# zzbuzzard/PATHS

Measured on AMD Instinct MI355X. Metric: slides_per_sec_5level_K2048_D1024, higher is better.
Workload: dtype f32 (products as 2 fp16 planes per operand = 22 bits, 3 fp16 MFMAs per block, fp32 accumulate); 1 GPU; 5-level PATHS recursion (forward, eval): K=2048 patches/level (level-0 grid 32x64, top_k 512, 10% background), D=1024 features, trans_dim 128 x 4 heads x 2 layers, LSTM ctx 256; 8 HBM-resident slides per GPU; slides_per_gpu=8, global_batch=8, levels=5, resident_batches_rotated=3, parallelism=slide-sharded x1 (no data-path collective)

## Files before the change

### paths_amd/csrc/gemm_epi.h

```cpp
#pragma once
#include "common.h"

namespace paths_epi {



struct TileView {
  char* base; int64_t ldb; uint32_t lane_off;
  __device__ TileView(const float* p, int64_t ld, int lane)
      : base(reinterpret_cast<char*>(const_cast<float*>(p))), ldb(ld * 4), lane_off((uint32_t)((4 * (lane >> 5)) * ld + (lane & 31)) * 4u) {}
  __device__ float* at(int trow, int tcol, int r) const {
    char* tile = base + (int64_t)trow * ldb + (int64_t)tcol * 4;
    const uint32_t off = lane_off + (uint32_t)((r & 3) + 8 * (r >> 2)) * (uint32_t)ldb;
    return reinterpret_cast<float*>(tile + off);
  }
  __device__ char* tile(int trow, int tcol) const { return base + (int64_t)trow * ldb + (int64_t)tcol * 4; }
  __device__ float* elem(char* tile_origin, int r) const {
    return reinterpret_cast<float*>(tile_origin + (lane_off + (uint32_t)((r & 3) + 8 * (r >> 2)) * (uint32_t)ldb));
  }
  __device__ float* at_clamped(int trow, int tcol, int r, int lane, int M) const {
    const int row = min(trow + c32_row(r, lane), M - 1);
    return reinterpret_cast<float*>(base + (int64_t)row * ldb + (int64_t)(tcol + (lane & 31)) * 4);
  }
};
template <bool FULL>
__device__ __forceinline__ float* tile_elem(const TileView& v, int trow, int tcol, int r, int lane, int M) {
  if constexpr (FULL) return v.at(trow, tcol, r);
  else return v.at_clamped(trow, tcol, r, lane, M);
}
template <bool FULL>
__device__ __forceinline__ float* tile_elem_o(const TileView& v, char* origin, int trow, int tcol, int r, int lane, int M) {
  if constexpr (FULL) return v.elem(origin, r);
  else return v.at_clamped(trow, tcol, r, lane, M);
}
template <bool FULL>
__device__ __forceinline__ bool tile_row_ok(int trow, int r, int lane, int M) {
  if constexpr (FULL) return true;
  else return trow + c32_row(r, lane) < M;
}

struct EpiLstmC {
  const float* bias;
  const float* c0; int64_t ldc0;
  float* c1; int64_t ldc1;
  float* frm; int64_t ldfrm;
  const float* hp; int64_t ldhp; const int* hp_row;
  float acc_scale = 1.0f;
  template <int WTM, int WTN>
  __device__ __forceinline__ void init(f32x16 (&acc)[WTM][WTN], int row0, int col0, int lane, int M) const {
    const int jj = lane & 31;
    const float seed = 1.0f / acc_scale;
    if (hp == nullptr) {
#pragma unroll
      for (int i = 0; i < WTM; ++i)
#pragma unroll
        for (int r = 0; r < 16; ++r) { acc[i][0][r] = 0.f; acc[i][1][r] = 0.f; acc[i][2][r] = 0.f; }
      return;
    }
    int pr[WTM][16];
#pragma unroll
    for (int i = 0; i < WTM; ++i)
#pragma unroll
      for (int r = 0; r < 16; ++r) pr[i][r] = hp_row[min(row0 + 32 * i + c32_row(r, lane), M - 1)];
    float t[2][3][16];
    auto issue = [&](auto ic) __attribute__((always_inline)) {
      constexpr int i = decltype(ic)::value;
#pragma unroll
      for (int r = 0; r < 16; ++r) {
        const float* ph = hp + (int64_t)max(pr[i][r], 0) * ldhp + col0 + jj;
        t[i & 1][0][r] = ph[0]; t[i & 1][1][r] = ph[32]; t[i & 1][2][r] = ph[64];
      }
    };
    issue(std::integral_constant<int, 0>{});
    static_for<0, WTM>([&](auto ic) __attribute__((always_inline)) {
      constexpr int i = decltype(ic)::value;
      __builtin_amdgcn_sched_barrier(0);
      if constexpr (i + 1 < WTM) issue(std::integral_constant<int, i + 1>{});
      __builtin_amdgcn_sched_barrier(0);
#pragma unroll
      for (int r = 0; r < 16; ++r) {
        const bool has = pr[i][r] >= 0;
        acc[i][0][r] = has ? t[i & 1][0][r] * seed : 0.f; acc[i][1][r] = has ? t[i & 1][1][r] * seed : 0.f; acc[i][2][r] = has ? t[i & 1][2][r] * seed : 0.f;
      }
    });
    __builtin_amdgcn_sched_barrier(0);
  }
  template <bool FULL, bool WITH_FRM, int WTM, int WTN>
  __device__ __forceinline__ void run_impl(f32x16 (&acc)[WTM][WTN], int row0, int col0, int lane, int M) const {
    const int jj = lane & 31;
    const int tcol = (col0 / 96) * 32;
    const float bf = bias[col0 + jj], br = bias[col0 + 32 + jj], bm = bias[col0 + 64 + jj];
    const TileView c0v(c0, ldc0, lane), c1v(c1, ldc1, lane), fv(frm, ldfrm, lane);
    static_for<0, WTM>([&](auto ic) __attribute__((always_inline)) {
      constexpr int i = decltype(ic)::value;
      const int trow = row0 + 32 * i;
      char* o0 = c0v.tile(trow, tcol); char* o1 = c1v.tile(trow, tcol); char* of = fv.tile(trow, col0);
      float cp[16];
#pragma unroll
      for (int r = 0; r < 16; ++r) cp[r] = c0 ? *tile_elem_o<FULL>(c0v, o0, trow, tcol, r, lane, M) : 0.f;
#pragma unroll
      for (int r = 0; r < 16; ++r) {
        const float f = sigmoid_acc(fmaf(acc[i][0][r], acc_scale, bf));
        const float rg = sigmoid_acc(fmaf(acc[i][1][r], acc_scale, br));
        const float mp = tanh_acc(fmaf(acc[i][2][r], acc_scale, bm));
        const float v = cp[r] * f + rg * mp;
        if (tile_row_ok<FULL>(trow, r, lane, M)) {
          *tile_elem_o<FULL>(c1v, o1, trow, tcol, r, lane, M) = v;
          if constexpr (WITH_FRM) {
            float* fr = tile_elem_o<FULL>(fv, of, trow, col0, r, lane, M);
            fr[0] = f; fr[32] = rg; fr[64] = mp;
          }
        }
      }
      __builtin_amdgcn_sched_barrier(0);
    });
  }
  template <int WTM, int WTN, int WGM, int WGN>
  __device__ __forceinline__ void run(f32x16 (&acc)[WTM][WTN], int row0, int col0, int lane, int, int, int M, float*) const {
    static_assert(WTN == 3, "LSTM c epilogue wants f|r|m tiles");
    const bool full = row0 + 32 * WTM <= M;
    if (frm == nullptr) {
      if (full) run_impl<true, false>(acc, row0, col0, lane, M);
      else run_impl<false, false>(acc, row0, col0, lane, M);
    } else {
      if (full) run_impl<true, true>(acc, row0, col0, lane, M);
      else run_impl<false, true>(acc, row0, col0, lane, M);
    }
  }
};

template <bool RAW>
struct EpiLstmO_ {
  const float* bias; float* o; int64_t ldo; int N;
  const float* hp; int64_t ldhp; const int* hp_row; int hp_col0;
  float acc_scale = 1.0f;
  template <int WTM, int WTN>
  __device__ __forceinline__ void init(f32x16 (&acc)[WTM][WTN], int row0, int col0, int lane, int M) const {
    const float seed = 1.0f / acc_scale;
    if (hp == nullptr) {
#pragma unroll
      for (int i = 0; i < WTM; ++i)
#pragma unroll
        for (int j = 0; j < WTN; ++j)
#pragma unroll
          for (int r = 0; r < 16; ++r) acc[i][j][r] = 0.f;
      return;
    }
    int pr[WTM][16];
#pragma unroll
    for (int i = 0; i < WTM; ++i)
#pragma unroll
      for (int r = 0; r < 16; ++r) pr[i][r] = hp_row[min(row0 + 32 * i + c32_row(r, lane), M - 1)];
    float t[2][WTN][16];
    auto issue = [&](auto ic) __attribute__((always_inline)) {
      constexpr int i = decltype(ic)::value;
#pragma unroll
      for (int r = 0; r < 16; ++r) {
        const float* ph = hp + (int64_t)max(pr[i][r], 0) * ldhp + hp_col0 + (lane & 31);
#pragma unroll
        for (int j = 0; j < WTN; ++j) t[i & 1][j][r] = ph[min(col0 + 32 * j, N - 32)];
      }
    };
    issue(std::integral_constant<int, 0>{});
    static_for<0, WTM>([&](auto ic) __attribute__((always_inline)) {
      constexpr int i = decltype(ic)::value;
      __builtin_amdgcn_sched_barrier(0);
      if constexpr (i + 1 < WTM) issue(std::integral_constant<int, i + 1>{});
      __builtin_amdgcn_sched_barrier(0);
#pragma unroll
      for (int r = 0; r < 16; ++r)
#pragma unroll
        for (int j = 0; j < WTN; ++j) acc[i][j][r] = pr[i][r] >= 0 ? t[i & 1][j][r] * seed : 0.f;
    });
    __builtin_amdgcn_sched_barrier(0);
  }
  template <bool FULL, int WTM, int WTN>
  __device__ __forceinline__ void run_impl(f32x16 (&acc)[WTM][WTN], int row0, int col0, int lane, int M) const {
    const TileView ov(o, ldo, lane);
    static_for<0, WTM * WTN>([&](auto tc) __attribute__((always_inline)) {
      constexpr int t = decltype(tc)::value, i = t % WTM, j = t / WTM;
      const int trow = row0 + 32 * i, tcol = col0 + 32 * j;
      if (tcol < N) {
        const float b = bias[tcol + (lane & 31)];
        char* origin = ov.tile(trow, tcol);
#pragma unroll
        for (int r = 0; r < 16; ++r) {
          const float v = sigmoid_acc(fmaf(acc[i][j][r], acc_scale, b));
          if (tile_row_ok<FULL>(trow, r, lane, M)) *tile_elem_o<FULL>(ov, origin, trow, tcol, r, lane, M) = v;
        }
      }
    });
  }
  template <int WTM, int WTN, int WGM, int WGN>
  __device__ __forceinline__ void run(f32x16 (&acc)[WTM][WTN], int row0, int col0, int lane, int, int, int M, float*) const {
    if constexpr (RAW) {
      const int ntn = N >> 5;
#pragma unroll
      for (int j = 0; j < WTN; ++j) {
        const int tcol = col0 + 32 * j;
        if (tcol < N) {
          const float b = bias[tcol + (lane & 31)];
#pragma unroll
          for (int i = 0; i < WTM; ++i) {
            f32x4* t = reinterpret_cast<f32x4*>(o + ((int64_t)((row0 >> 5) + i) * ntn + (tcol >> 5)) * 1024) + lane;
#pragma unroll
            for (int q = 0; q < 4; ++q)
              t[64 * q] = f32x4{fmaf(acc[i][j][4 * q], acc_scale, b), fmaf(acc[i][j][4 * q + 1], acc_scale, b),
                                fmaf(acc[i][j][4 * q + 2], acc_scale, b), fmaf(acc[i][j][4 * q + 3], acc_scale, b)};
          }
        }
      }
    } else {
      if (row0 + 32 * WTM <= M) run_impl<true>(acc, row0, col0, lane, M);
      else run_impl<false>(acc, row0, col0, lane, M);
    }
  }
};
typedef EpiLstmO_<false> EpiLstmO;
typedef EpiLstmO_<true> EpiLstmORaw;

template <bool WITH_Y, bool WITH_TC = false, bool RAW_O = false>
struct EpiLstmH {
  template <int WTM, int WTN>
  __device__ __forceinline__ void init(f32x16 (&acc)[WTM][WTN], int, int, int, int) const {
#pragma unroll
    for (int i = 0; i < WTM; ++i)
#pragma unroll
      for (int j = 0; j < WTN; ++j)
#pragma unroll
        for (int r = 0; r < 16; ++r) acc[i][j][r] = 0.f;
  }

  const float* bias; const float* o; int64_t ldo; const float* x; int64_t ldx;
  float* h1; int64_t ldh; float* y; int64_t ldy; int N;
  float* tc_out;
  float acc_scale = 1.0f;
  template <bool FULL, int WTM, int WTN>
  __device__ __forceinline__ void run_impl(f32x16 (&acc)[WTM][WTN], int row0, int col0, int lane, int M) const {
    constexpr int NT = WTM * WTN, PD = (NT >= 4 && !WITH_Y) ? 3 : 1, NB = PD + 1;
    const TileView ovw(o, ldo, lane), xvw(x, ldx, lane), hv(h1, ldh, lane), yv(y, ldy, lane), tv(tc_out, N, lane);
    float ov[NB][16], xv[WITH_Y ? NB : 1][16];
    auto load = [&](auto tc) __attribute__((always_inline)) {
      constexpr int t = decltype(tc)::value, i = t % WTM, j = t / WTM, s = t % NB;
      const int trow = row0 + 32 * i, tcol = min(col0 + 32 * j, N - 32);
      char* to = ovw.tile(trow, tcol); char* tx = xvw.tile(trow, tcol);
      if constexpr (RAW_O) {
        const f32x4* t4 = reinterpret_cast<const f32x4*>(o + ((int64_t)(trow >> 5) * (N >> 5) + (tcol >> 5)) * 1024) + lane;
#pragma unroll
        for (int q = 0; q < 4; ++q) {
          const f32x4 v = t4[64 * q];
          ov[s][4 * q] = v[0]; ov[s][4 * q + 1] = v[1]; ov[s][4 * q + 2] = v[2]; ov[s][4 * q + 3] = v[3];
        }
      }
      static_for<0, 16>([&](auto rc) __attribute__((always_inline)) {
        constexpr int r = decltype(rc)::value;
        if constexpr (FULL) {
          if constexpr (!RAW_O) ov[s][r] = *ovw.elem(to, r);
          if constexpr (WITH_Y) xv[s][r] = *xvw.elem(tx, r);
        } else {
          if constexpr (!RAW_O) ov[s][r] = *ovw.at_clamped(trow, tcol, r, lane, M);
          if constexpr (WITH_Y) xv[s][r] = *xvw.at_clamped(trow, tcol, r, lane, M);
        }
      });
    };
    static_for<0, (PD < NT ? PD : NT)>([&](auto tc) __attribute__((always_inline)) { load(tc); });
    static_for<0, NT>([&](auto tc) __attribute__((always_inline)) {
      constexpr int t = decltype(tc)::value, i = t % WTM, j = t / WTM, s = t % NB;
      if constexpr (t + PD < NT) load(std::integral_constant<int, t + PD>{});
      const int trow = row0 + 32 * i, tcol = col0 + 32 * j;
      if (tcol < N) {
        const float b = bias[tcol + (lane & 31)];
        char* th = hv.tile(trow, tcol); char* ty = yv.tile(trow, tcol); char* tt = tv.tile(trow, tcol);
        static_for<0, 16>([&](auto rc) __attribute__((always_inline)) {
          constexpr int r = decltype(rc)::value;
          const float tcv = tanh_acc(fmaf(acc[i][j][r], acc_scale, b));
          const float h = (RAW_O ? sigmoid_acc(ov[s][r]) : ov[s][r]) * tcv;
          if constexpr (FULL) {
            if constexpr (WITH_TC) *tv.elem(tt, r) = tcv;
            *hv.elem(th, r) = h;
            if constexpr (WITH_Y) *yv.elem(ty, r) = xv[s][r] + h;
          } else if (tile_row_ok<false>(trow, r, lane, M)) {
            if constexpr (WITH_TC) *tv.at_clamped(trow, tcol, r, lane, M) = tcv;
            *hv.at_clamped(trow, tcol, r, lane, M) = h;
            if constexpr (WITH_Y) *yv.at_clamped(trow, tcol, r, lane, M) = xv[s][r] + h;
          }
        });
      }
      __builtin_amdgcn_sched_barrier(0);
    });
  }
  template <int WTM, int WTN, int WGM, int WGN>
  __device__ __forceinline__ void run(f32x16 (&acc)[WTM][WTN], int row0, int col0, int lane, int, int, int M, float*) const {
    if (row0 + 32 * WTM <= M) run_impl<true>(acc, row0, col0, lane, M);
    else run_impl<false>(acc, row0, col0, lane, M);
  }
};

struct EpiBias {
  template <int WTM, int WTN>
  __device__ __forceinline__ void init(f32x16 (&acc)[WTM][WTN], int, int, int, int) const {
#pragma unroll
    for (int i = 0; i < WTM; ++i)
#pragma unroll
      for (int j = 0; j < WTN; ++j)
#pragma unroll
        for (int r = 0; r < 16; ++r) acc[i][j][r] = 0.f;
  }

  const float* bias; float* out; int64_t ldo; int N; int act;
  const float* residual; int64_t ldr; const float* mask; int64_t ldm; int accumulate;
  float acc_scale = 1.0f;
  template <bool FULL, int WTM, int WTN>
  __device__ __forceinline__ void run_impl(f32x16 (&acc)[WTM][WTN], int row0, int col0, int lane, int M) const {
    constexpr int NT = WTM * WTN;
    const TileView outv(out, ldo, lane), resv(residual, ldr, lane), maskv(mask, ldm, lane);
    float rv[2][16], mv[2][16], ov[2][16];
    const bool any_load = residual != nullptr || mask != nullptr || accumulate != 0;
    auto load = [&](auto tc) __attribute__((always_inline)) {
      constexpr int t = decltype(tc)::value, i = t % WTM, j = t / WTM, s = t & 1;
      const int trow = row0 + 32 * i, tcol = col0 + 32 * j;
      const int lcol = min(tcol + (lane & 31), N - 1) - (lane & 31);
#pragma unroll
      for (int r = 0; r < 16; ++r) {
        rv[s][r] = residual ? *tile_elem<FULL>(resv, trow, lcol, r, lane, M) : 0.f;
        mv[s][r] = mask ? *tile_elem<FULL>(maskv, trow, lcol, r, lane, M) : 1.f;
        ov[s][r] = accumulate ? *tile_elem<FULL>(outv, trow, lcol, r, lane, M) : 0.f;
      }
    };
    if (any_load) load(std::integral_constant<int, 0>{});
    static_for<0, NT>([&](auto tc) __attribute__((always_inline)) {
      constexpr int t = decltype(tc)::value, i = t % WTM, j = t / WTM, s = t & 1;
      if constexpr (t + 1 < NT) {
        if (any_load) load(std::integral_constant<int, t + 1>{});
      }
      const int trow = row0 + 32 * i, tcol = col0 + 32 * j;
      const int colr = tcol + (lane & 31);
      const float b = bias ? bias[min(colr, N - 1)] : 0.f;
      if (tcol < N) {
#pragma unroll
        for (int r = 0; r < 16; ++r) {
          float v = fmaf(acc[i][j][r], acc_scale, b);
          if (act == 1) v = fmaxf(v, 0.f);
          if (any_load) {
            if (!(mv[s][r] > 0.f)) v = 0.f;
            v += rv[s][r] + ov[s][r];
          }
          if (tile_row_ok<FULL>(trow, r, lane, M) && (tcol + 32 <= N || colr < N)) *tile_elem<FULL>(outv, trow, tcol, r, lane, M) = v;
        }
      }
      __builtin_amdgcn_sched_barrier(0);
    });
  }
  template <int WTM, int WTN, int WGM, int WGN>
  __device__ __forceinline__ void run(f32x16 (&acc)[WTM][WTN], int row0, int col0, int lane, int, int, int M, float*) const {
    if (row0 + 32 * WTM <= M) run_impl<true>(acc, row0, col0, lane, M);
    else run_impl<false>(acc, row0, col0, lane, M);
  }
};

__device__ __forceinline__ int div_u24(int x, int d, float rd) {
  int q = (int)((float)x * rd);
  const int r = x - q * d;
  q += (r >= d) - (r < 0);
  return q;
}
__device__ __forceinline__ int div_pos(int64_t x, int d, float rd) {
  return (x >= 0 && x < (1 << 24)) ? div_u24((int)x, d, rd) : (int)(x / d);
}

template <bool PE_TAB, bool SAVE = false>
struct EpiImpProj {
  template <int WTM, int WTN>
  __device__ __forceinline__ void init(f32x16 (&acc)[WTM][WTN], int, int, int, int) const {
#pragma unroll
    for (int i = 0; i < WTM; ++i)
#pragma unroll
      for (int j = 0; j < WTN; ++j)
#pragma unroll
        for (int r = 0; r < 16; ++r) acc[i][j][r] = 0.f;
  }

  const float* b1; const float* w2; const float* b2;
  const float* bp;
  const float* special;
  const float* div_term;
  const int64_t* locs;
  const int64_t* num_ims;
  int rows_per_slide;
  int patch_size;
  int pe_mode;
  int imp_mul;
  float* importance;
  float* tokens;
  float* hid_out;
  float* pproj_out;
  const float* pe_table; int pe_rows;
  float acc_scale = 1.0f;
  template <int WTM, int WTN, int WGM, int WGN>
  __device__ __forceinline__ void run(f32x16 (&acc)[WTM][WTN], int row0, int col0, int lane, int wm, int wn, int M, float* smem) const {
    static_assert(WTN == 4 && WGN == 2, "imp/proj epilogue layout: one block spans the 128 hidden + 128 projected columns");
    constexpr int d = 128, RB = WGM * WTM * 32;
    const float rps_inv = 1.0f / (float)rows_per_slide, ps_inv = 1.0f / (float)patch_size;
    const bool small_rows = M < (1 << 24);
    const int u0 = 64 * wn;
    float* alpha_p = smem;
#pragma unroll
    for (int i = 0; i < WTM; ++i) {
      float part[16];
#pragma unroll
      for (int r = 0; r < 16; ++r) part[r] = 0.f;
#pragma unroll
      for (int j = 0; j < 2; ++j) {
        const int u = u0 + 32 * j + (lane & 31);
        const float b = b1[u], w = w2[u];
#pragma unroll
        for (int r = 0; r < 16; ++r) {
          const float hv = fmaxf(fmaf(acc[i][j][r], acc_scale, b), 0.f);
          part[r] += hv * w;
          const int row = row0 + 32 * i + c32_row(r, lane);
          if constexpr (SAVE) { if (row < M) hid_out[(int64_t)row * 128 + u] = hv; }
        }
      }
      float p8[8], p4[4], p2[2], p1;
      {
        const bool up = (lane & 16) != 0;
#pragma unroll
        for (int k = 0; k < 8; ++k) {
          const float keep = up ? part[8 + k] : part[k], send = up ? part[k] : part[8 + k];
          p8[k] = keep + __shfl_xor(send, 16);
        }
      }
      {
        const bool up = (lane & 8) != 0;
#pragma unroll
        for (int k = 0; k < 4; ++k) {
          const float keep = up ? p8[4 + k] : p8[k], send = up ? p8[k] : p8[4 + k];
          p4[k] = keep + __shfl_xor(send, 8);
        }
      }
      {
        const bool up = (lane & 4) != 0;
#pragma unroll
        for (int k = 0; k < 2; ++k) {
          const float keep = up ? p4[2 + k] : p4[k], send = up ? p4[k] : p4[2 + k];
          p2[k] = keep + __shfl_xor(send, 4);
        }
      }
      {
        const bool up = (lane & 2) != 0;
        const float keep = up ? p2[1] : p2[0], send = up ? p2[0] : p2[1];
        p1 = keep + __shfl_xor(send, 2);
      }
      p1 += __shfl_xor(p1, 1);
      const int rho = (lane >> 1) & 15;
      if ((lane & 1) == 0) alpha_p[wn * RB + wm * WTM * 32 + 32 * i + c32_row(rho, lane)] = p1;
    }
    __syncthreads();
    const float b2v = *b2;
    float bpv[2], dtv[2], spv[2];
#pragma unroll
    for (int j = 0; j < 2; ++j) {
      const int c = u0 + 32 * j + (lane & 31);
      bpv[j] = bp[c];
      spv[j] = special[c];
      dtv[j] = pe_mode == 2 ? div_term[(c & (d / 2 - 1)) >> 1] : div_term[c >> 1];
    }
#pragma unroll
    for (int i = 0; i < WTM; ++i) {
      int64_t lp[16];
#pragma unroll
      for (int r = 0; r < 16; ++r) {
        const int rowc = min(row0 + 32 * i + c32_row(r, lane), M - 1);
        lp[r] = pe_mode == 2 ? locs[2 * (int64_t)rowc + wn] : 0;
      }
      const int trow0 = min(row0 + 32 * i, M - 1);
      const int b0 = small_rows ? div_u24(trow0, rows_per_slide, rps_inv) : trow0 / rows_per_slide, idx0 = trow0 - b0 * rows_per_slide;
      const int nslides = M / rows_per_slide;
      const int nim0 = (int)num_ims[b0], nim1 = (int)num_ims[min(b0 + 1, nslides - 1)];
      int tokrow[16]; float av[16]; bool first[16]; float pev[16][2];
#pragma unroll
      for (int r = 0; r < 16; ++r) {
        const int lrow = wm * WTM * 32 + 32 * i + c32_row(r, lane);
        const int rowr = row0 + 32 * i + c32_row(r, lane);
        int b, idx, nim;
        if (rows_per_slide >= 32) {
          const int off = min(rowr, M - 1) - trow0;
          const bool next = idx0 + off >= rows_per_slide;
          b = b0 + (next ? 1 : 0); idx = idx0 + off - (next ? rows_per_slide : 0); nim = next ? nim1 : nim0;
        } else {
          const int row = min(rowr, M - 1);
          b = small_rows ? div_u24(row, rows_per_slide, rps_inv) : row / rows_per_slide; idx = row - b * rows_per_slide; nim = (int)num_ims[b];
        }
        float a = 0.f;
        if (idx < nim) a = sigmoid_acc((alpha_p[lrow] + alpha_p[RB + lrow]) + b2v);
        if (wn == 0 && (lane & 31) == 0 && rowr < M) importance[rowr] = a;
        av[r] = imp_mul ? a : 1.f;
        tokrow[r] = b * (rows_per_slide + 1) + idx + 1;
        first[r] = idx == 0;
        if constexpr (PE_TAB) {
          const int px24 = (int)min(max(lp[r], (int64_t)0), (int64_t)((1 << 24) - 1));
          const int ipos = pe_mode == 2 ? div_u24(px24, patch_size, ps_inv) : idx;
          const int tp = min(ipos, pe_rows - 1);
#pragma unroll
          for (int j = 0; j < 2; ++j) {
            const int c = u0 + 32 * j + (lane & 31);
            pev[r][j] = pe_mode == 2 ? pe_table[(int64_t)tp * (d / 2) + (c & (d / 2 - 1))] : pe_table[(int64_t)tp * d + c];
          }
        } else {
          const int ipos = pe_mode == 2 ? div_pos(lp[r], patch_size, ps_inv) : idx;
#pragma unroll
          for (int j = 0; j < 2; ++j) {
            const int c = u0 + 32 * j + (lane & 31);
            const float ang = (float)ipos * dtv[j];
            pev[r][j] = (c & 1) ? cosf(ang) : sinf(ang);
          }
        }
      }
#pragma unroll
      for (int r = 0; r < 16; ++r) {
        const int row = row0 + 32 * i + c32_row(r, lane);
        if (row < M) {
          float* trow = tokens + (int64_t)tokrow[r] * d;
#pragma unroll
          for (int j = 0; j < 2; ++j) {
            const int c = u0 + 32 * j + (lane & 31);
            const float pj = acc[i][2 + j][r] * acc_scale;
            trow[c] = av[r] * pj + bpv[j] + pev[r][j];
            if constexpr (SAVE) pproj_out[(int64_t)row * 128 + c] = pj;
            if (first[r]) trow[c - d] = spv[j];
          }
        }
      }
    }
  }
};

}
```

### paths_amd/csrc/gemm_x6.hip

```cpp
#include "common.h"
#include "gemm_epi.h"
#include "finish_qkv.h"
#include "split.h"

#ifndef PATHS_X6_PART
#define PATHS_X6_PART 0
#endif

namespace {
using namespace paths_epi;

constexpr int FRAG = 1024;
template <int NP> constexpr int planes_of() { return NP == 4 ? 2 : NP; }
template <int NP> constexpr int subt() { return planes_of<NP>() * FRAG; }

struct X6Operands {
  const float* A0; int64_t lda0; int K0;
  const int64_t* A0rows;
  const float* A1; int64_t lda1; int K1;
  const float* Aadd; int64_t ldadd;
  const char* Wt;
  int64_t w_group_stride;
  int M;
  const int64_t* num_ims;
  int rows_per_slide;
  float a_scale;
  int ksplit = 1;
};

template <int NP, int WTM, int WTN, int PF, bool ADD, bool ROWS, class Epi, int OCC = 1, bool A16 = false>
__global__ void __launch_bounds__(256) __attribute__((amdgpu_waves_per_eu(OCC, OCC)))
gemm_x6_kernel(X6Operands g, Epi epi) {
  static_assert(NP == 2 || NP == 3 || NP == 4, "two fp16 planes, three bf16 planes or two bf16 planes");
  static_assert(!A16 || (NP == 2 && ROWS), "fp16 A rows: two-plane fp16 split, row-pointer form");
  constexpr int PL = planes_of<NP>();
  constexpr bool A1P = A16 && !ADD;
  constexpr int PLA = A1P ? 1 : PL;
  constexpr int SUBT = subt<NP>();
  constexpr int SUBTA = PLA * FRAG;
  constexpr int NPROD = NP == 3 ? 6 : A1P ? 2 : 3;
  constexpr int BM = WTM * 64, BN = WTN * 64;
  constexpr int SA = 2 * WTM, SB = 2 * WTN;
  constexpr int STAGE = SA * SUBTA + SB * SUBT;
  constexpr int NA = BM / 64;
  constexpr int NPB = SB * PL, NB = (NPB + 3) / 4;
  static_assert(WTM % 2 == 0, "A fragment register slots alternate per accumulator row");
  extern __shared__ __attribute__((aligned(16))) char smem[];
  const int tid = threadIdx.x, lane = tid & 63, wave = __builtin_amdgcn_readfirstlane(tid >> 6), wm = wave >> 1, wn = wave & 1;

  const int nbx = gridDim.x, nby = gridDim.y, nblk = nbx * nby;
  const int lin = xcd_tile_order(blockIdx.y * nbx + blockIdx.x, nblk);
  constexpr int GM = 8;
  const int per_group = GM * nbx;
  const int grp = lin / per_group, in_grp = lin - grp * per_group;
  const int rows_in_grp = min(GM, nby - grp * GM);
  const int by = grp * GM + in_grp % rows_in_grp, bx = in_grp / rows_in_grp;
  const int m0 = by * BM, n0 = bx * BN;
  if (block_all_padding(g.num_ims, g.rows_per_slide, m0, BM, g.M)) return;

  const int arow = tid >> 2, ac = tid & 3;
  uint32_t aoff0[NA], aoff1[NA], aoffs[ADD ? NA : 1]; int awr[NA];
  typedef const f32x4 __attribute__((address_space(1))) * gptr_f4;
  typedef const u32x2 __attribute__((address_space(1))) * gptr_h4;
  gptr_f4 rowp[ROWS && !A16 ? NA : 1];
  gptr_h4 rowh[A16 ? NA : 1];
#pragma unroll
  for (int p = 0; p < NA; ++p) {
    const int row = p * 64 + arow;
    const int64_t grow = min(m0 + row, g.M - 1);
    aoff0[p] = ROWS ? 0u : (uint32_t)((grow * g.lda0 + 4 * ac) * 4);
    if constexpr (A16) rowh[p] = reinterpret_cast<gptr_h4>(static_cast<uintptr_t>(g.A0rows[grow]) + 8 * ac);
    else if constexpr (ROWS) rowp[p] = reinterpret_cast<gptr_f4>(static_cast<uintptr_t>(g.A0rows[grow]) + 16 * ac);
    aoff1[p] = (uint32_t)((grow * g.lda1 + 4 * ac) * 4);
    if constexpr (ADD) aoffs[p] = (uint32_t)((grow * g.ldadd + 4 * ac) * 4);
    awr[p] = (row >> 5) * SUBTA + (ac >> 1) * 512 + (row & 31) * 16 + (ac & 1) * 8;
  }
  const int K0w = g.ksplit > 1 ? g.K0 / g.ksplit : g.K0;
  const int kofs = g.ksplit > 1 ? (int)blockIdx.z * K0w : 0;
  if (kofs != 0) {
#pragma unroll
    for (int p = 0; p < NA; ++p) {
      aoff0[p] += (uint32_t)kofs * 4u;
      if constexpr (A16) rowh[p] += kofs >> 2;
      else if constexpr (ROWS) rowp[p] += kofs >> 2;
      if constexpr (ADD) aoffs[p] += (uint32_t)kofs * 4u;
    }
  }
  const int nk0 = K0w >> 4, nk = (K0w + g.K1) >> 4;
  const char* bbase[NB]; int bwr[NB];
#pragma unroll
  for (int i = 0; i < NB; ++i) {
    int pc = wave + 4 * i;
    if (pc >= NPB) pc -= 4;
    const int sub = pc / PL, pl = pc % PL;
    bbase[i] = g.Wt + ((int64_t)(n0 >> 5) + sub) * g.w_group_stride + pl * FRAG;
    bwr[i] = (A1P ? SA * SUBTA + sub * SUBT : (SA + sub) * SUBT) + pl * FRAG + lane * 16;
  }
  static_assert(PF == 1 || PF == 2, "one or two register sets");
  f32x4 sa[PF][NA], sadd[ADD ? PF : 1][ADD ? NA : 1]; u32x4 sbr[PF][NB];
  u32x2 sh[A16 ? PF : 1][A16 ? NA : 1];
  uint32_t hi[NA][2], mid[NP != 2 ? NA : 1][2], lo[NA][2];
  float* const anyA = const_cast<float*>(ROWS ? reinterpret_cast<const float*>(g.Wt) : g.A0);
  const auto rsA0 = __builtin_amdgcn_make_buffer_rsrc(anyA, 0, 0xFFFFFFFFu, 0x00020000);
  const auto rsA1 = __builtin_amdgcn_make_buffer_rsrc(g.A1 ? const_cast<float*>(g.A1) : anyA, 0, 0xFFFFFFFFu, 0x00020000);
  const auto rsAdd = __builtin_amdgcn_make_buffer_rsrc(ADD ? const_cast<float*>(g.Aadd) : anyA, 0, 0xFFFFFFFFu, 0x00020000);
  const auto rsW = __builtin_amdgcn_make_buffer_rsrc(const_cast<char*>(g.Wt), 0, 0xFFFFFFFFu, 0x00020000);
  const int lane16 = lane * 16;
  int bsoff[NB];
#pragma unroll
  for (int i = 0; i < NB; ++i) bsoff[i] = (int)(bbase[i] - g.Wt) + (kofs >> 4) * SUBT;
  auto gload_a = [&](int set, int q, int kt) {
    const bool first = kt < nk0;
    const int soff = (first ? kt : kt - nk0) * 64;
    if constexpr (A16) {
      sh[set][q] = rowh[q][kt * 4];
    } else if constexpr (ROWS) {
      sa[set][q] = rowp[q][kt * 4];
    } else {
      const u32x4 raw = first ? __builtin_amdgcn_raw_buffer_load_b128(rsA0, (int)aoff0[q], soff, 0)
                              : __builtin_amdgcn_raw_buffer_load_b128(rsA1, (int)aoff1[q], soff, 0);
      sa[set][q] = __builtin_bit_cast(f32x4, raw);
    }
    if constexpr (ADD) {
      sadd[set][q] = __builtin_bit_cast(f32x4, __builtin_amdgcn_raw_buffer_load_b128(rsAdd, (int)aoffs[q], kt * 64, 0));
    }
  };
  auto gload_b = [&](int set, int q, int kt) {
    sbr[set][q] = __builtin_amdgcn_raw_buffer_load_b128(rsW, lane16, bsoff[q] + kt * SUBT, 0);
  };
  constexpr int PRE = ADD ? (A16 ? 2 : 1) : 0;
  constexpr int NS = A1P ? 2 : (NP == 3 ? 12 : NP == 4 ? 7 : 5) + PRE;
  float tf[NA][2];
  const uint32_t s2 = A1P ? __builtin_bit_cast(uint32_t, f16x2{(_Float16)g.a_scale, (_Float16)g.a_scale}) : 0u;
  auto a_step = [&](int set, int q, int st0, int buf) __attribute__((always_inline)) {
    f32x4& v = sa[set][q];
    const int st = st0 - PRE;
    if constexpr (ADD && A16) {
      if (st0 == 0) { v[0] = h_lo(sh[set][q][0]) + sadd[set][q][0]; v[1] = h_hi(sh[set][q][0]) + sadd[set][q][1]; }
      if (st0 == 1) { v[2] = h_lo(sh[set][q][1]) + sadd[set][q][2]; v[3] = h_hi(sh[set][q][1]) + sadd[set][q][3]; }
    } else if constexpr (ADD) {
      if (st0 == 0) v += sadd[set][q];
    }
    if constexpr (A1P) {
      if (st == 0) {
        asm("v_pk_mul_f16 %0, %1, %2" : "=v"(hi[q][0]) : "v"(sh[set][q][0]), "v"(s2));
        asm("v_pk_mul_f16 %0, %1, %2" : "=v"(hi[q][1]) : "v"(sh[set][q][1]), "v"(s2));
      }
      if (st == 1) *reinterpret_cast<u32x2*>(smem + buf * STAGE + awr[q]) = u32x2{hi[q][0], hi[q][1]};
    } else if constexpr (NP == 3) {
      if (st == 0) { hi[q][0] = pk_bf16(v[0], v[1]); hi[q][1] = pk_bf16(v[2], v[3]); }
      if (st == 1) { tf[q][0] = bf_lo(hi[q][0]); tf[q][1] = bf_hi(hi[q][0]); }
      if (st == 2) { v[0] -= tf[q][0]; v[1] -= tf[q][1]; }
      if (st == 3) { tf[q][0] = bf_lo(hi[q][1]); tf[q][1] = bf_hi(hi[q][1]); }
      if (st == 4) { v[2] -= tf[q][0]; v[3] -= tf[q][1]; }
      if (st == 5) { mid[q][0] = pk_bf16(v[0], v[1]); mid[q][1] = pk_bf16(v[2], v[3]); }
      if (st == 6) { tf[q][0] = bf_lo(mid[q][0]); tf[q][1] = bf_hi(mid[q][0]); }
      if (st == 7) { v[0] -= tf[q][0]; v[1] -= tf[q][1]; }
      if (st == 8) { tf[q][0] = bf_lo(mid[q][1]); tf[q][1] = bf_hi(mid[q][1]); }
      if (st == 9) { v[2] -= tf[q][0]; v[3] -= tf[q][1]; }
      if (st == 10) { lo[q][0] = pk_bf16(v[0], v[1]); lo[q][1] = pk_bf16(v[2], v[3]); }
      if (st == 11) {
        char* d = smem + buf * STAGE + awr[q];
        *reinterpret_cast<u32x2*>(d) = u32x2{hi[q][0], hi[q][1]};
        *reinterpret_cast<u32x2*>(d + FRAG) = u32x2{mid[q][0], mid[q][1]};
        *reinterpret_cast<u32x2*>(d + 2 * FRAG) = u32x2{lo[q][0], lo[q][1]};
      }
    } else if constexpr (NP == 4) {
      if (st == 0) { hi[q][0] = pk_bf16(v[0], v[1]); hi[q][1] = pk_bf16(v[2], v[3]); }
      if (st == 1) { tf[q][0] = bf_lo(hi[q][0]); tf[q][1] = bf_hi(hi[q][0]); }
      if (st == 2) { v[0] -= tf[q][0]; v[1] -= tf[q][1]; }
      if (st == 3) { tf[q][0] = bf_lo(hi[q][1]); tf[q][1] = bf_hi(hi[q][1]); }
      if (st == 4) { v[2] -= tf[q][0]; v[3] -= tf[q][1]; }
      if (st == 5) { mid[q][0] = pk_bf16(v[0], v[1]); mid[q][1] = pk_bf16(v[2], v[3]); }
      if (st == 6) {
        char* d = smem + buf * STAGE + awr[q];
        *reinterpret_cast<u32x2*>(d) = u32x2{hi[q][0], hi[q][1]};
        *reinterpret_cast<u32x2*>(d + FRAG) = u32x2{mid[q][0], mid[q][1]};
      }
    } else {
      if (st == 0) v *= g.a_scale;
      if (st == 1) { hi[q][0] = pk_f16(v[0], v[1]); hi[q][1] = pk_f16(v[2], v[3]); }
      if (st == 2) {
        asm("v_fma_mixlo_f16 %0, %1, -1.0, %2 op_sel_hi:[1,0,0]" : "=v"(lo[q][0]) : "v"(hi[q][0]), "v"(v[0]));
        asm("v_fma_mixlo_f16 %0, %1, -1.0, %2 op_sel_hi:[1,0,0]" : "=v"(lo[q][1]) : "v"(hi[q][1]), "v"(v[2]));
      }
      if (st == 3) {
        asm("v_fma_mixhi_f16 %0, %1, -1.0, %2 op_sel:[1,0,0] op_sel_hi:[1,0,0]" : "+v"(lo[q][0]) : "v"(hi[q][0]), "v"(v[1]));
        asm("v_fma_mixhi_f16 %0, %1, -1.0, %2 op_sel:[1,0,0] op_sel_hi:[1,0,0]" : "+v"(lo[q][1]) : "v"(hi[q][1]), "v"(v[3]));
      }
      if (st == 4) {
        char* d = smem + buf * STAGE + awr[q];
        *reinterpret_cast<u32x2*>(d) = u32x2{hi[q][0], hi[q][1]};
        *reinterpret_cast<u32x2*>(d + FRAG) = u32x2{lo[q][0], lo[q][1]};
      }
    }
  };
  auto swrite_b = [&](int set, int q, int buf) { *reinterpret_cast<u32x4*>(smem + buf * STAGE + bwr[q]) = sbr[set][q]; };

  f32x16 acc[WTM][WTN];
  epi.template init<WTM, WTN>(acc, m0 + wm * WTM * 32, n0 + wn * WTN * 32, lane, g.M);

  const char* sA = smem + (wm * WTM) * SUBTA + lane * 16;
  const char* sB = A1P ? smem + SA * SUBTA + (wn * WTN) * SUBT + lane * 16 : smem + (SA + wn * WTN) * SUBT + lane * 16;
  u32x4 fa[2][PLA], fb[2][WTN][PL];
  auto read_a = [&](int buf, int i, int slot, int p) { fa[slot][p] = *reinterpret_cast<const u32x4*>(sA + buf * STAGE + i * SUBTA + p * FRAG); };
  auto read_b = [&](int buf, int j, int slot, int p) { fb[slot][j][p] = *reinterpret_cast<const u32x4*>(sB + buf * STAGE + j * SUBT + p * FRAG); };
  constexpr int RG = WTN * NPROD;
  auto one_mfma = [&](int gq, int sb) __attribute__((always_inline)) {
    const int i = gq / RG, j = (gq % RG) / NPROD, t = gq % NPROD, sl = i & 1;
    if constexpr (NP == 3) {
      constexpr int PA_[6] = {2, 0, 1, 1, 0, 0}, PB_[6] = {0, 2, 1, 0, 1, 0};
      acc[i][j] = __builtin_amdgcn_mfma_f32_32x32x16_bf16(__builtin_bit_cast(bf16x8, fa[sl][PA_[t]]), __builtin_bit_cast(bf16x8, fb[sb][j][PB_[t]]), acc[i][j], 0, 0, 0);
    } else if constexpr (NP == 4) {
      constexpr int PA_[3] = {1, 0, 0}, PB_[3] = {0, 1, 0};
      acc[i][j] = __builtin_amdgcn_mfma_f32_32x32x16_bf16(__builtin_bit_cast(bf16x8, fa[sl][PA_[t]]), __builtin_bit_cast(bf16x8, fb[sb][j][PB_[t]]), acc[i][j], 0, 0, 0);
    } else if constexpr (A1P) {
      constexpr int PB_[2] = {1, 0};
      acc[i][j] = __builtin_amdgcn_mfma_f32_32x32x16_f16(__builtin_bit_cast(f16x8, fa[sl][0]), __builtin_bit_cast(f16x8, fb[sb][j][PB_[t]]), acc[i][j], 0, 0, 0);
    } else {
      constexpr int PA_[3] = {1, 0, 0}, PB_[3] = {0, 1, 0};
      acc[i][j] = __builtin_amdgcn_mfma_f32_32x32x16_f16(__builtin_bit_cast(f16x8, fa[sl][PA_[t]]), __builtin_bit_cast(f16x8, fb[sb][j][PB_[t]]), acc[i][j], 0, 0, 0);
    }
  };
  constexpr int AG = (WTM - 1) * RG;
  constexpr auto fits = [](int spg) constexpr {
    return PF == 1 ? ((NS + spg - 1) / spg) * NA + NB <= AG : (NS * NA + spg - 1) / spg + NB <= AG;
  };
  constexpr int SPG = fits(1) ? 1 : fits(2) ? 2 : fits(3) ? 3 : 4;
  static_assert(fits(SPG), "staging does not fit before the barrier");
  constexpr int GPC = (NS + SPG - 1) / SPG;
  constexpr int GA2 = (NS * NA + SPG - 1) / SPG;
  constexpr int TS = PF == 1 ? GPC * NA + NB : GA2 + NB + NA + NB;
  static_assert(TS <= WTM * RG, "staging does not fit in a stage");
  constexpr int AR0 = RG / 2;
  auto staging_slot = [&](auto sc, int kt, auto bufc, auto m1c, auto m2c) __attribute__((always_inline)) {
    constexpr int s = decltype(sc)::value, buf = decltype(bufc)::value;
    constexpr bool more1 = decltype(m1c)::value, more2 = decltype(m2c)::value;
    constexpr int set = PF == 2 ? (buf ^ 1) : 0;
    if constexpr (PF == 1) {
      if constexpr (s < GPC * NA) {
        constexpr int q = s / GPC, g0 = s % GPC;
        if constexpr (more1) {
          static_for<g0 * SPG, (g0 + 1) * SPG < NS ? (g0 + 1) * SPG : NS>([&](auto mc) __attribute__((always_inline)) {
            a_step(set, q, decltype(mc)::value, buf ^ 1);
          });
        }
        if constexpr (more2 && g0 == GPC - 1) gload_a(set, q, kt + 1 + PF);
      } else if constexpr (s < TS) {
        if constexpr (more1) swrite_b(set, s - GPC * NA, buf ^ 1);
        if constexpr (more2) gload_b(set, s - GPC * NA, kt + 1 + PF);
      }
    } else {
      if constexpr (s < GA2) {
        if constexpr (more1) {
          static_for<s * SPG, (s + 1) * SPG < NS * NA ? (s + 1) * SPG : NS * NA>([&](auto mc) __attribute__((always_inline)) {
            constexpr int m = decltype(mc)::value;
            a_step(set, m / NS, m % NS, buf ^ 1);
          });
        }
      } else if constexpr (s < GA2 + NB) {
        if constexpr (more1) swrite_b(set, s - GA2, buf ^ 1);
      } else if constexpr (s < GA2 + NB + NA) {
        if constexpr (more2) gload_a(set, s - GA2 - NB, kt + 1 + PF);
      } else if constexpr (s < TS) {
        if constexpr (more2) gload_b(set, s - GA2 - NB - NA, kt + 1 + PF);
      }
    }
  };
  auto stage_body = [&](int kt, auto bufc, auto m1c, auto m2c) __attribute__((always_inline)) {
    constexpr int buf = decltype(bufc)::value, sb = buf;
    constexpr bool more1 = decltype(m1c)::value, more2 = decltype(m2c)::value;
    constexpr int set = PF == 2 ? (buf ^ 1) : 0;
    static_for<0, AG>([&](auto gc) __attribute__((always_inline)) {
      constexpr int gq = decltype(gc)::value, i = gq / RG, gr = gq % RG;
      one_mfma(gq, sb);
      if constexpr (gr >= AR0 && gr < AR0 + PLA) read_a(buf, i + 1, (i + 1) & 1, gr - AR0);
      staging_slot(std::integral_constant<int, gq>{}, kt, bufc, m1c, m2c);
      __builtin_amdgcn_sched_barrier(0);
    });
    __syncthreads();
    __builtin_amdgcn_sched_barrier(0);
    static_for<AG, WTM * RG>([&](auto gc) __attribute__((always_inline)) {
      constexpr int gq = decltype(gc)::value, gr = gq % RG;
      one_mfma(gq, sb);
      if constexpr (more1) {
        static_for<2 * gr, 2 * gr + 2>([&](auto fc) __attribute__((always_inline)) {
          constexpr int f = decltype(fc)::value;
          if constexpr (f < PLA) read_a(buf ^ 1, 0, 0, f);
          else if constexpr (f < PLA + PL * WTN) read_b(buf ^ 1, (f - PLA) / PL, sb ^ 1, (f - PLA) % PL);
        });
      }
      staging_slot(std::integral_constant<int, gq>{}, kt, bufc, m1c, m2c);
      __builtin_amdgcn_sched_barrier(0);
    });
  };
  constexpr std::integral_constant<int, 0> I0{};
  constexpr std::integral_constant<int, 1> I1{};
  constexpr std::true_type T{};
  constexpr std::false_type F{};

#pragma unroll
  for (int q = 0; q < NA; ++q) gload_a(0, q, 0);
#pragma unroll
  for (int q = 0; q < NB; ++q) gload_b(0, q, 0);
#pragma unroll
  for (int q = 0; q < NA; ++q)
#pragma unroll
    for (int st = 0; st < NS; ++st) a_step(0, q, st, 0);
#pragma unroll
  for (int q = 0; q < NB; ++q) swrite_b(0, q, 0);
#pragma unroll
  for (int sidx = 1; sidx <= PF; ++sidx) {
#pragma unroll
    for (int q = 0; q < NA; ++q) gload_a(PF == 2 ? (sidx & 1) : 0, q, sidx);
#pragma unroll
    for (int q = 0; q < NB; ++q) gload_b(PF == 2 ? (sidx & 1) : 0, q, sidx);
  }
  __syncthreads();
#pragma unroll
  for (int p = 0; p < PLA; ++p) read_a(0, 0, 0, p);
#pragma unroll
  for (int j = 0; j < WTN; ++j)
#pragma unroll
    for (int p = 0; p < PL; ++p) read_b(0, j, 0, p);
  for (int kt = 0; kt < nk - 2 * PF; kt += 2) {
    __builtin_amdgcn_sched_barrier(0);
    stage_body(kt, I0, T, T);
    stage_body(kt + 1, I1, T, T);
  }
  if constexpr (PF == 2) {
    stage_body(nk - 4, I0, T, T);
    stage_body(nk - 3, I1, T, F);
  }
  stage_body(nk - 2, I0, T, F);
  stage_body(nk - 1, I1, F, F);
  __syncthreads();
  epi.template run<WTM, WTN, 2, 2>(acc, m0 + wm * WTM * 32, n0 + wn * WTN * 32, lane, wm, wn, g.M, reinterpret_cast<float*>(smem));
}

template <int NP>
__global__ void x6_pack_kernel(const float* __restrict__ w, int64_t ldw, uint16_t* __restrict__ out, int N, int Npad, int K, float wscale) {
  const int64_t i = blockIdx.x * (int64_t)blockDim.x + threadIdx.x;
  if (i >= (int64_t)Npad * K) return;
  const int n = (int)(i / K), k = (int)(i % K);
  const float v = n < N ? w[(int64_t)n * ldw + k] * wscale : 0.f;
  uint16_t* o = out + ((int64_t)(n >> 5) * (K >> 4) + (k >> 4)) * (subt<NP>() / 2) + ((k >> 3) & 1) * 256 + (n & 31) * 8 + (k & 7);
  if constexpr (NP == 3) {
    const __bf16 h = (__bf16)v; const float r1 = v - (float)h;
    const __bf16 m = (__bf16)r1; const float r2 = r1 - (float)m;
    const __bf16 l = (__bf16)r2;
    o[0] = __builtin_bit_cast(uint16_t, h); o[FRAG / 2] = __builtin_bit_cast(uint16_t, m); o[FRAG] = __builtin_bit_cast(uint16_t, l);
  } else if constexpr (NP == 4) {
    const __bf16 h = (__bf16)v; const float r1 = v - (float)h;
    const __bf16 m = (__bf16)r1;
    o[0] = __builtin_bit_cast(uint16_t, h); o[FRAG / 2] = __builtin_bit_cast(uint16_t, m);
  } else {
    const _Float16 h = (_Float16)v; const float r1 = v - (float)h;
    const _Float16 l = (_Float16)r1;
    o[0] = __builtin_bit_cast(uint16_t, h); o[FRAG / 2] = __builtin_bit_cast(uint16_t, l);
  }
}

template <int NP>
__global__ void x6_pack_t_kernel(const float* __restrict__ w, int64_t ldw, uint16_t* __restrict__ out, int N, int Npad, int K, int Kvalid) {
  static_assert(NP == 3 || NP == 4, "bf16 planes (scale 1)");
  const int64_t i = blockIdx.x * (int64_t)blockDim.x + threadIdx.x;
  if (i >= (int64_t)Npad * (K >> 3)) return;
  const int n = (int)(i % Npad), k0 = (int)(i / Npad) * 8;
  uint16_t h[8], m[8], l[8];
#pragma unroll
  for (int j = 0; j < 8; ++j) {
    const int k = k0 + j;
    const float v = (n < N && k < Kvalid) ? w[(int64_t)k * ldw + n] : 0.f;
    const __bf16 hh = (__bf16)v; const float r1 = v - (float)hh;
    const __bf16 mm = (__bf16)r1; const float r2 = r1 - (float)mm;
    const __bf16 ll = (__bf16)r2;
    h[j] = __builtin_bit_cast(uint16_t, hh); m[j] = __builtin_bit_cast(uint16_t, mm); l[j] = __builtin_bit_cast(uint16_t, ll);
  }
  uint16_t* o = out + ((int64_t)(n >> 5) * (K >> 4) + (k0 >> 4)) * (subt<NP>() / 2) + ((k0 >> 3) & 1) * 256 + (n & 31) * 8;
  typedef uint16_t u16x8 __attribute__((ext_vector_type(8)));
  *reinterpret_cast<u16x8*>(o) = u16x8{h[0], h[1], h[2], h[3], h[4], h[5], h[6], h[7]};
  *reinterpret_cast<u16x8*>(o + FRAG / 2) = u16x8{m[0], m[1], m[2], m[3], m[4], m[5], m[6], m[7]};
  if constexpr (NP == 3) *reinterpret_cast<u16x8*>(o + FRAG) = u16x8{l[0], l[1], l[2], l[3], l[4], l[5], l[6], l[7]};
}

template <int NP, int WTM, int WTN, int PF, bool ADD, bool ROWS, class Epi, int OCC = 1, bool A16 = false>
int launch_x6_np(const X6Operands& g, int Npad, const Epi& epi, hipStream_t stream, const char* name) {
  constexpr int BM = WTM * 64, BN = WTN * 64;
  constexpr size_t lds = 2ull * (2 * WTM * ((A16 && !ADD) ? FRAG : subt<NP>()) + 2 * WTN * subt<NP>());
  const int K = g.K0 + g.K1;
  PATHS_REQUIRE(g.M > 0, "%s: M must be > 0", name);
  PATHS_REQUIRE(g.K0 > 0 && g.K0 % 16 == 0 && g.K1 % 16 == 0 && K % 32 == 0 && K >= 128, "%s: K panels (%d,%d): multiples of 16, total a multiple of 32, >= 128", name, g.K0, g.K1);
  PATHS_REQUIRE(Npad % BN == 0, "%s: packed N (%d) must be a multiple of %d", name, Npad, BN);
  PATHS_REQUIRE(g.lda0 % 4 == 0 && g.lda1 % 4 == 0, "%s: leading dims must be multiples of 4 floats", name);
  PATHS_REQUIRE(((uintptr_t)g.A0 % 16 == 0) && ((uintptr_t)g.A1 % 16 == 0) && ((uintptr_t)g.Wt % 16 == 0), "%s: operands must be 16-byte aligned", name);
  PATHS_REQUIRE(ROWS == (g.A0rows != nullptr) && (!ROWS || g.K1 == 0), "%s: row-pointer form is single-panel", name);
  PATHS_REQUIRE((int64_t)g.M * (g.lda0 > g.lda1 ? (g.lda0 > g.ldadd ? g.lda0 : g.ldadd) : (g.lda1 > g.ldadd ? g.lda1 : g.ldadd)) * 4 < (int64_t)1 << 32, "%s: A panel larger than 4 GiB", name);
  auto kern = gemm_x6_kernel<NP, WTM, WTN, PF, ADD, ROWS, Epi, OCC, A16>;
  PATHS_LDS_OPT_IN(kern, lds, name);
  PATHS_REQUIRE(g.ksplit == 1 || (g.ksplit > 1 && g.K1 == 0 && g.K0 % (32 * g.ksplit) == 0 && g.K0 / g.ksplit >= 128), "%s: split-K needs a single panel and k windows that are multiples of 32, >= 128", name);
  dim3 grid(Npad / BN, (g.M + BM - 1) / BM, g.ksplit);
  hipLaunchKernelGGL(kern, grid, dim3(256), lds, stream, g, epi);
  PATHS_LAUNCH_CHECK(name);
  return PATHS_OK;
}

struct EpiRaw {
  float* ws; int64_t zstride; int ntn;
  template <int WTM, int WTN>
  __device__ __forceinline__ void init(f32x16 (&acc)[WTM][WTN], int, int, int, int) const {
#pragma unroll
    for (int i = 0; i < WTM; ++i)
#pragma unroll
      for (int j = 0; j < WTN; ++j)
#pragma unroll
        for (int r = 0; r < 16; ++r) acc[i][j][r] = 0.f;
  }
  template <int WTM, int WTN, int WGM, int WGN>
  __device__ __forceinline__ void run(f32x16 (&acc)[WTM][WTN], int row0, int col0, int lane, int, int, int, float*) const {
    float* base = ws + (int64_t)blockIdx.z * zstride;
#pragma unroll
    for (int i = 0; i < WTM; ++i)
#pragma unroll
      for (int j = 0; j < WTN; ++j) {
        f32x4* t = reinterpret_cast<f32x4*>(base + ((int64_t)((row0 >> 5) + i) * ntn + (col0 >> 5) + j) * 1024) + lane;
#pragma unroll
        for (int q = 0; q < 4; ++q) {
          const f32x4 v = f32x4{acc[i][j][4 * q], acc[i][j][4 * q + 1], acc[i][j][4 * q + 2], acc[i][j][4 * q + 3]};
          t[64 * q] = v;
        }
      }
  }
};

template <int NZ, class Epi>
__global__ void __launch_bounds__(256)
x6_finish_kernel(const float* __restrict__ ws, int64_t zstride, int ntn, int M, const int64_t* __restrict__ num_ims, int rows_per_slide, Epi epi) {
  extern __shared__ __attribute__((aligned(16))) char smem[];
  const int tid = threadIdx.x, lane = tid & 63, wave = __builtin_amdgcn_readfirstlane(tid >> 6), wm = wave >> 1, wn = wave & 1;
  const int m0 = blockIdx.x * 64;
  if (block_all_padding(num_ims, rows_per_slide, m0, 64, M)) return;
  const int row0 = m0 + wm * 32, col0 = wn * 128;
  f32x16 acc[1][4];
#pragma unroll
  for (int j = 0; j < 4; ++j) {
    const f32x4* t = reinterpret_cast<const f32x4*>(ws + ((int64_t)(row0 >> 5) * ntn + (col0 >> 5) + j) * 1024) + lane;
#pragma unroll
    for (int q = 0; q < 4; ++q) {
      f32x4 v = t[64 * q];
#pragma unroll
      for (int z = 1; z < NZ; ++z) v += *reinterpret_cast<const f32x4*>(reinterpret_cast<const float*>(t + 64 * q) + z * zstride);
      acc[0][j][4 * q] = v[0]; acc[0][j][4 * q + 1] = v[1]; acc[0][j][4 * q + 2] = v[2]; acc[0][j][4 * q + 3] = v[3];
    }
  }
  epi.template run<1, 4, 2, 2>(acc, row0, col0, lane, wm, wn, M, reinterpret_cast<float*>(smem));
}

template <int WTM, int WTN, int PF, bool ADD, class Epi>
int launch_x6(int planes, const X6Operands& g, int Npad, const Epi& epi, hipStream_t stream, const char* name) {
  if (g.A0rows != nullptr) {
    if (planes == 2) return launch_x6_np<2, WTM, WTN, PF, ADD, true>(g, Npad, epi, stream, name);
    return paths_set_error(PATHS_EUNSUPPORTED, "%s: row pointers need planes = 2", name);
  }
  if constexpr (std::is_same<Epi, EpiBias>::value && !ADD) {
    if (planes == 4) return launch_x6_np<4, WTM, WTN, PF, ADD, false>(g, Npad, epi, stream, name);
  }
  if (planes == 3) return launch_x6_np<3, WTM, WTN, PF, ADD, false>(g, Npad, epi, stream, name);
  if (planes == 2) return launch_x6_np<2, WTM, WTN, PF, ADD, false>(g, Npad, epi, stream, name);
  return paths_set_error(PATHS_EINVAL, "%s: planes must be 3 (bf16 x6) or 2 (fp16 x3), got %d", name, planes);
}

constexpr int H_OCC = 3;
constexpr int H_TRAIN_OCC = 2;

inline int plane_count(int planes) { return planes == 4 ? 2 : planes; }
inline int64_t group_stride(int planes, int Kpacked) { return (int64_t)(Kpacked / 16) * plane_count(planes) * FRAG; }
inline bool pow2(float x) { int e; return x > 0.f && frexpf(x, &e) == 0.5f; }
inline bool h16_scale_ok(float a_scale) { return pow2(a_scale) && a_scale >= 1.0f && a_scale <= 32768.0f; }

}

extern "C" {

#if PATHS_X6_PART == 0 || PATHS_X6_PART == 1
int64_t paths_x6_packed_bytes(int Npad, int K, int planes) { return (int64_t)Npad * K * 2 * plane_count(planes); }

int paths_x6_pack_weights(const float* w, int64_t ldw, void* out, int N, int Npad, int K, int planes, float w_scale, hipStream_t stream) {
  PATHS_REQUIRE(N > 0 && Npad >= N && Npad % 32 == 0 && K % 16 == 0, "x6_pack_weights: bad shape N=%d Npad=%d K=%d", N, Npad, K);
  PATHS_REQUIRE((uintptr_t)out % 16 == 0, "x6_pack_weights: out must be 16-byte aligned");
  PATHS_REQUIRE(((planes == 3 || planes == 4) && w_scale == 1.0f) || (planes == 2 && pow2(w_scale)), "x6_pack_weights: planes 3 / 4 (bf16) with w_scale 1, or planes 2 with a power-of-two w_scale");
  const int64_t n = (int64_t)Npad * K;
  const dim3 grid((unsigned)((n + 255) / 256));
  if (planes == 4) hipLaunchKernelGGL(x6_pack_kernel<4>, grid, dim3(256), 0, stream, w, ldw, reinterpret_cast<uint16_t*>(out), N, Npad, K, 1.0f);
  else if (planes == 3) hipLaunchKernelGGL(x6_pack_kernel<3>, grid, dim3(256), 0, stream, w, ldw, reinterpret_cast<uint16_t*>(out), N, Npad, K, 1.0f);
  else hipLaunchKernelGGL(x6_pack_kernel<2>, grid, dim3(256), 0, stream, w, ldw, reinterpret_cast<uint16_t*>(out), N, Npad, K, w_scale);
  PATHS_LAUNCH_CHECK("x6_pack_weights");
  return PATHS_OK;
}

int paths_x6_pack_weights_t(const float* w, int64_t ldw, void* out, int N, int Npad, int K, int Kvalid, int planes, hipStream_t stream) {
  PATHS_REQUIRE(N > 0 && Npad >= N && Npad % 32 == 0 && K % 16 == 0 && Kvalid > 0 && Kvalid <= K, "x6_pack_weights_t: bad shape N=%d Npad=%d K=%d Kvalid=%d", N, Npad, K, Kvalid);
  PATHS_REQUIRE(w != nullptr && out != nullptr && (uintptr_t)out % 16 == 0, "x6_pack_weights_t: null / unaligned operand");
  PATHS_REQUIRE(planes == 3 || planes == 4, "x6_pack_weights_t: planes 3 or 4 (bf16)");
  const int64_t n = (int64_t)Npad * (K / 8);
  const dim3 grid((unsigned)((n + 255) / 256));
  if (planes == 4) hipLaunchKernelGGL(x6_pack_t_kernel<4>, grid, dim3(256), 0, stream, w, ldw, reinterpret_cast<uint16_t*>(out), N, Npad, K, Kvalid);
  else hipLaunchKernelGGL(x6_pack_t_kernel<3>, grid, dim3(256), 0, stream, w, ldw, reinterpret_cast<uint16_t*>(out), N, Npad, K, Kvalid);
  PATHS_LAUNCH_CHECK("x6_pack_weights_t");
  return PATHS_OK;
}

}
namespace {
template <bool A16>
int lstm_cell_x6(const float* x, int64_t ldx, const int64_t* x_rows, const float* h0, int64_t ldh0, const float* c0, int64_t ldc0,
                 const void* w_gates_x6, const float* b_gates, const void* w_mem_x6, const float* b_mem,
                 float* state_out, int64_t ldso, float* y, int64_t ldy, float* ws_o, float* save_frm, float* save_tc,
                 const float* hp, const int* hp_row, int M, int D, int Hc, const int64_t* num_ims, int rows_per_slide,
                 int phases, int planes, float wg_scale, float wm_scale, float a_scale, hipStream_t stream) {
  PATHS_REQUIRE(D % 256 == 0 && Hc % 64 == 0, "lstm_cell_x6: D (%d) must be a multiple of 256 and Hc (%d) of 64", D, Hc);
  if constexpr (A16) {
    PATHS_REQUIRE(x_rows != nullptr && x == nullptr && planes == 2, "lstm_cell_x6_h16: fp16 rows are given as x_rows (planes = 2)");
    PATHS_REQUIRE(h16_scale_ok(a_scale), "lstm_cell_x6_h16: a_scale must be a power of two in [1, 2^15]");
  }
  PATHS_REQUIRE(hp != nullptr || (h0 == nullptr) == (c0 == nullptr), "lstm_cell_x6: h0 and c0 must both be given or both be null");
  PATHS_REQUIRE((hp == nullptr) == (hp_row == nullptr) && (hp == nullptr || h0 == nullptr),
                "lstm_cell_x6: hp/hp_row come together and replace h0 (the h half of the gate GEMM was done per parent)");
  PATHS_REQUIRE(planes == 3 || (pow2(wg_scale) && pow2(wm_scale) && pow2(a_scale)), "lstm_cell_x6: scales must be powers of two");
  PATHS_REQUIRE(x_rows == nullptr || (h0 == nullptr && y == nullptr && save_tc == nullptr), "lstm_cell_x6: x_rows (rows addressed in place) excludes h0, y and the training saves");
  if (planes == 3) wg_scale = wm_scale = a_scale = 1.0f;
  const char* wg = reinterpret_cast<const char*>(w_gates_x6);
  const int64_t gs = group_stride(planes, 2 * D);
  const float sg = 1.0f / (wg_scale * a_scale), sm = 1.0f / (wm_scale * a_scale);
  X6Operands g{x, ldx, D, x_rows, h0, h0 ? ldh0 : 0, h0 ? D : 0, nullptr, 0, wg, gs, M, num_ims, rows_per_slide, a_scale};
  const bool small_m = planes == 2 && M <= 8192 && (h0 == nullptr);
  if (phases & 1) {
    EpiLstmC e{b_gates, c0, ldc0, state_out + D, ldso, save_frm, (int64_t)3 * Hc, hp, (int64_t)3 * Hc + D, hp_row, sg};
    int rc;
    if constexpr (A16) {
      rc = small_m ? launch_x6_np<2, 2, 3, 2, false, true, decltype(e), 1, true>(g, 3 * Hc, e, stream, "lstm_cell_x6_h16(c, 128-row tiles)")
                   : launch_x6_np<2, 4, 3, 1, false, true, decltype(e), 1, true>(g, 3 * Hc, e, stream, "lstm_cell_x6_h16(c)");
    } else if (small_m) rc = x_rows ? launch_x6_np<2, 2, 3, 2, false, true>(g, 3 * Hc, e, stream, "lstm_cell_x6(c, 128-row tiles)")
                             : launch_x6_np<2, 2, 3, 2, false, false>(g, 3 * Hc, e, stream, "lstm_cell_x6(c, 128-row tiles)");
    else rc = launch_x6<4, 3, 1, false>(planes, g, 3 * Hc, e, stream, "lstm_cell_x6(c)");
    if (rc) return rc;
  }
  const bool o_raw = y == nullptr && save_tc == nullptr && save_frm == nullptr;
  if (phases & 2) {
    X6Operands go = g;
    go.Wt = wg + (int64_t)(3 * Hc / 32) * gs;
    int rc;
    if (o_raw) {
      EpiLstmORaw e{b_gates + 3 * Hc, ws_o, D, D, hp, (int64_t)3 * Hc + D, hp_row, 3 * Hc, sg};
      if constexpr (A16) {
        rc = small_m ? launch_x6_np<2, 2, 4, 2, false, true, decltype(e), 1, true>(go, D, e, stream, "lstm_cell_x6_h16(o, raw, 128-row tiles)")
                     : launch_x6_np<2, 4, 4, 1, false, true, decltype(e), 1, true>(go, D, e, stream, "lstm_cell_x6_h16(o, raw)");
      } else if (small_m) rc = x_rows ? launch_x6_np<2, 2, 4, 2, false, true>(go, D, e, stream, "lstm_cell_x6(o, raw, 128-row tiles)")
                               : launch_x6_np<2, 2, 4, 2, false, false>(go, D, e, stream, "lstm_cell_x6(o, raw, 128-row tiles)");
      else rc = launch_x6<4, 4, 1, false>(planes, go, D, e, stream, "lstm_cell_x6(o, raw)");
    } else {
      EpiLstmO e{b_gates + 3 * Hc, ws_o, D, D, hp, (int64_t)3 * Hc + D, hp_row, 3 * Hc, sg};
      if constexpr (A16) rc = launch_x6_np<2, 4, 4, 1, false, true, decltype(e), 1, true>(go, D, e, stream, "lstm_cell_x6_h16(o)");
      else rc = launch_x6<4, 4, 1, false>(planes, go, D, e, stream, "lstm_cell_x6(o)");
    }
    if (rc) return rc;
  }
  if (phases & 4) {
    X6Operands gh{state_out + D, ldso, Hc, nullptr, nullptr, 0, 0, nullptr, 0, reinterpret_cast<const char*>(w_mem_x6), group_stride(planes, Hc), M, num_ims, rows_per_slide, a_scale};
    int rc;
    PATHS_REQUIRE(save_tc == nullptr || y != nullptr, "lstm_cell_x6: save_tc (training) needs y");
    PATHS_REQUIRE(planes == 2 || planes == 3, "lstm_cell_x6: planes must be 3 (bf16 x6) or 2 (fp16 x3), got %d", planes);
    if (save_tc != nullptr) {
      EpiLstmH<true, true> e{b_mem, ws_o, D, x, ldx, state_out, ldso, y, ldy, D, save_tc, sm};
      if (planes == 2) rc = launch_x6_np<2, 2, 2, 2, false, false, decltype(e), H_TRAIN_OCC>(gh, D, e, stream, "lstm_cell_x6(h, save, 128x128)");
      else rc = launch_x6_np<3, 4, 4, 1, false, false>(gh, D, e, stream, "lstm_cell_x6(h, save)");
    } else if (y != nullptr) {
      EpiLstmH<true, false> e{b_mem, ws_o, D, x, ldx, state_out, ldso, y, ldy, D, nullptr, sm};
      rc = launch_x6<4, 4, 1, false>(planes, gh, D, e, stream, "lstm_cell_x6(h)");
    } else if (o_raw) {
      EpiLstmH<false, false, true> e{b_mem, ws_o, D, x, ldx, state_out, ldso, nullptr, 0, D, nullptr, sm};
      if (planes == 2) rc = launch_x6_np<2, 2, 2, 2, false, false, decltype(e), H_OCC>(gh, D, e, stream, "lstm_cell_x6(h, raw o, 128x128)");
      else rc = launch_x6_np<3, 4, 4, 1, false, false>(gh, D, e, stream, "lstm_cell_x6(h, raw o)");
    } else {
      EpiLstmH<false, false> e{b_mem, ws_o, D, x, ldx, state_out, ldso, nullptr, 0, D, nullptr, sm};
      if (planes == 2) rc = launch_x6_np<2, 2, 2, 2, false, false, decltype(e), H_OCC>(gh, D, e, stream, "lstm_cell_x6(h, no y, 128x128)");
      else rc = launch_x6_np<3, 4, 4, 1, false, false>(gh, D, e, stream, "lstm_cell_x6(h, no y)");
    }
    if (rc) return rc;
  }
  return PATHS_OK;
}
}
extern "C" {

int paths_lstm_cell_x6(const float* x, int64_t ldx, const int64_t* x_rows, const float* h0, int64_t ldh0, const float* c0, int64_t ldc0,
                       const void* w_gates_x6, const float* b_gates, const void* w_mem_x6, const float* b_mem,
                       float* state_out, int64_t ldso, float* y, int64_t ldy, float* ws_o, float* save_frm, float* save_tc,
                       const float* hp, const int* hp_row, int M, int D, int Hc, const int64_t* num_ims, int rows_per_slide,
                       int phases, int planes, float wg_scale, float wm_scale, float a_scale, hipStream_t stream) {
  return lstm_cell_x6<false>(x, ldx, x_rows, h0, ldh0, c0, ldc0, w_gates_x6, b_gates, w_mem_x6, b_mem, state_out, ldso, y, ldy, ws_o, save_frm,
                             save_tc, hp, hp_row, M, D, Hc, num_ims, rows_per_slide, phases, planes, wg_scale, wm_scale, a_scale, stream);
}

int paths_lstm_cell_x6_h16(const float* x, int64_t ldx, const int64_t* x_rows, const float* h0, int64_t ldh0, const float* c0, int64_t ldc0,
                           const void* w_gates_x6, const float* b_gates, const void* w_mem_x6, const float* b_mem,
                           float* state_out, int64_t ldso, float* y, int64_t ldy, float* ws_o, float* save_frm, float* save_tc,
                           const float* hp, const int* hp_row, int M, int D, int Hc, const int64_t* num_ims, int rows_per_slide,
                           int phases, int planes, float wg_scale, float wm_scale, float a_scale, hipStream_t stream) {
  return lstm_cell_x6<true>(x, ldx, x_rows, h0, ldh0, c0, ldc0, w_gates_x6, b_gates, w_mem_x6, b_mem, state_out, ldso, y, ldy, ws_o, save_frm,
                            save_tc, hp, hp_row, M, D, Hc, num_ims, rows_per_slide, phases, planes, wg_scale, wm_scale, a_scale, stream);
}

#endif
#if PATHS_X6_PART == 0 || PATHS_X6_PART == 2
int64_t paths_importance_proj_x6_workspace(int M) { return 2ll * ((M + 127) / 128 * 4) * 8 * 1024 * 4; }

}
namespace {
template <bool A16>
int importance_proj_x6(const float* y, int64_t ldy, const int64_t* y_rows, const float* y_add, int64_t ldya, const void* w_ip_x6, const float* b1, const float* w2, const float* b2,
                       const float* bp, const float* special, const float* div_term, const float* pe_table, int pe_rows, const int64_t* locs,
                       const int64_t* num_ims, int rows_per_slide, int patch_size, int pe_mode, int imp_mul,
                       float* importance, float* tokens, float* save_hid, float* save_pproj, int M, int D, int Hi, int d,
                       int skip_padding, int planes, float w_scale, float a_scale, float* splitk_ws, hipStream_t stream) {
  if constexpr (A16) {
    PATHS_REQUIRE(y == nullptr && y_rows != nullptr && y_add != nullptr && splitk_ws != nullptr && planes == 2 && D % 64 == 0 && D >= 256,
                  "importance_proj_x6_h16: fp16 rows (y_rows) + y_add on the split-K form (splitk_ws, planes = 2, D %% 64 == 0, D >= 256)");
  }
  PATHS_REQUIRE(Hi == 128 && d == 128, "importance_proj_x6: this build supports importance_mlp_hidden_dim=128, trans_dim=128 (got %d, %d)", Hi, d);
  PATHS_REQUIRE(pe_mode == 1 || pe_mode == 2, "importance_proj_x6: pe_mode must be 1 (1d) or 2 (2d)");
  PATHS_REQUIRE(pe_mode == 1 || locs != nullptr, "importance_proj_x6: 2d positional encoding needs locs");
  PATHS_REQUIRE(num_ims != nullptr && rows_per_slide > 0 && M % rows_per_slide == 0, "importance_proj_x6: bad slide layout");
  PATHS_REQUIRE(b1 != nullptr && w2 != nullptr && b2 != nullptr, "importance_proj_x6: b1, w2 and b2 (device scalar) are required");
  PATHS_REQUIRE(y_add == nullptr || (ldya % 4 == 0 && (uintptr_t)y_add % 16 == 0), "importance_proj_x6: y_add must be 16-byte aligned with ldya %% 4 == 0");
  PATHS_REQUIRE(planes == 3 || (pow2(w_scale) && pow2(a_scale)), "importance_proj_x6: scales must be powers of two");
  if (planes == 3) w_scale = a_scale = 1.0f;
  const float sc = 1.0f / (w_scale * a_scale);
  X6Operands g{y, ldy, D, y_rows, nullptr, 0, 0, y_add, ldya, reinterpret_cast<const char*>(w_ip_x6), group_stride(planes, D), M, skip_padding ? num_ims : nullptr, rows_per_slide, a_scale};
  PATHS_REQUIRE((save_hid == nullptr) == (save_pproj == nullptr), "importance_proj_x6: save_hid and save_pproj come together");
  PATHS_REQUIRE(pe_table == nullptr || pe_rows > 0, "importance_proj_x6: pe_rows must be > 0 with a pe_table");
  auto go = [&](auto epi) {
    decltype(epi) e{b1, w2, b2, bp, special, div_term, locs, num_ims, rows_per_slide, patch_size, pe_mode, imp_mul, importance, tokens,
                    save_hid, save_pproj, pe_table, pe_table ? pe_rows : 0, sc};
    {
      if (splitk_ws != nullptr && planes == 2 && (y_add != nullptr || y_rows == nullptr) && D % 64 == 0 && D >= 256) {
        const int mt = (M + 127) / 128 * 4;
        const int64_t zstride = (int64_t)mt * 8 * 1024;
        int rc;
        if constexpr (A16) {
          X6Operands gs = g; gs.ksplit = 2;
          EpiRaw raw{splitk_ws, zstride, 8};
          rc = launch_x6_np<2, 2, 4, 2, true, true, EpiRaw, 1, true>(gs, 256, raw, stream, "importance_proj_x6_h16(split-k)");
        } else {
          X6Operands gs = g; gs.ksplit = 2;
          EpiRaw raw{splitk_ws, zstride, 8};
          rc = y_add == nullptr ? launch_x6_np<2, 2, 4, 2, false, false>(gs, 256, raw, stream, "importance_proj_x6(split-k, stored y)")
               : y_rows ? launch_x6_np<2, 2, 4, 2, true, true>(gs, 256, raw, stream, "importance_proj_x6(split-k)")
                        : launch_x6_np<2, 2, 4, 2, true, false>(gs, 256, raw, stream, "importance_proj_x6(split-k)");
        }
        if (rc != PATHS_OK) return rc;
        const int fblk = (M + 63) / 64, fdepth = (fblk + 255) / 256;
        const int flds = fdepth == 1 ? 84 * 1024 : fdepth == 2 ? 54 * 1024 : fdepth == 3 ? 41 * 1024 : 1024;
        PATHS_LDS_OPT_IN((x6_finish_kernel<2, decltype(epi)>), 84 * 1024, "importance_proj_x6(finish)");
        PATHS_LAUNCH_STOP((x6_finish_kernel<2, decltype(epi)>), dim3(fblk), dim3(256), flds, stream, splitk_ws, zstride, 8, M,
                          skip_padding ? num_ims : nullptr, rows_per_slide, e);
        PATHS_LAUNCH_CHECK("importance_proj_x6(finish)");
        return PATHS_OK;
      }
    }
    if constexpr (A16) {
      return paths_set_error(PATHS_EUNSUPPORTED, "importance_proj_x6_h16: split-K form only");
    } else {
      if (y_add != nullptr) return launch_x6<2, 4, 2, true>(planes, g, 256, e, stream, "importance_proj_x6(sum)");
      return launch_x6<2, 4, 2, false>(planes, g, 256, e, stream, "importance_proj_x6");
    }
  };
  if (pe_table != nullptr) return save_hid ? go(EpiImpProj<true, true>{}) : go(EpiImpProj<true, false>{});
  return save_hid ? go(EpiImpProj<false, true>{}) : go(EpiImpProj<false, false>{});
}
}
extern "C" {

int paths_importance_proj_x6(const float* y, int64_t ldy, const int64_t* y_rows, const float* y_add, int64_t ldya, const void* w_ip_x6, const float* b1, const float* w2, const float* b2,
                             const float* bp, const float* special, const float* div_term, const float* pe_table, int pe_rows, const int64_t* locs,
                             const int64_t* num_ims, int rows_per_slide, int patch_size, int pe_mode, int imp_mul,
                             float* importance, float* tokens, float* save_hid, float* save_pproj, int M, int D, int Hi, int d,
                             int skip_padding, int planes, float w_scale, float a_scale, float* splitk_ws, hipStream_t stream) {
  return importance_proj_x6<false>(y, ldy, y_rows, y_add, ldya, w_ip_x6, b1, w2, b2, bp, special, div_term, pe_table, pe_rows, locs, num_ims,
                                   rows_per_slide, patch_size, pe_mode, imp_mul, importance, tokens, save_hid, save_pproj, M, D, Hi, d,
                                   skip_padding, planes, w_scale, a_scale, splitk_ws, stream);
}

int paths_importance_proj_x6_h16(const float* y, int64_t ldy, const int64_t* y_rows, const float* y_add, int64_t ldya, const void* w_ip_x6, const float* b1, const float* w2, const float* b2,
                                 const float* bp, const float* special, const float* div_term, const float* pe_table, int pe_rows, const int64_t* locs,
                                 const int64_t* num_ims, int rows_per_slide, int patch_size, int pe_mode, int imp_mul,
                                 float* importance, float* tokens, float* save_hid, float* save_pproj, int M, int D, int Hi, int d,
                                 int skip_padding, int planes, float w_scale, float a_scale, float* splitk_ws, hipStream_t stream) {
  return importance_proj_x6<true>(y, ldy, y_rows, y_add, ldya, w_ip_x6, b1, w2, b2, bp, special, div_term, pe_table, pe_rows, locs, num_ims,
                                  rows_per_slide, patch_size, pe_mode, imp_mul, importance, tokens, save_hid, save_pproj, M, D, Hi, d,
                                  skip_padding, planes, w_scale, a_scale, splitk_ws, stream);
}


}
namespace {
template <bool A16>
int importance_qkv_x6(const float* y, int64_t ldy, const int64_t* y_rows, const float* y_add, int64_t ldya, const void* w_ip_x6,
                      const float* b1, const float* w2, const float* b2, const float* bp, const float* special,
                      const float* pe_table, int pe_rows, const int64_t* locs, const int64_t* num_ims, int B, int N,
                      int patch_size, int pe_mode, int imp_mul, float* importance, float* tokens, int D, int skip_padding,
                      float w_scale, float a_scale, float* splitk_ws, const void* w_qkv, const float* bqkv, float s_wqkv,
                      float qscale, void* qkv_images, int phases, int alpha_from_importance, hipStream_t stream) {
  PATHS_REQUIRE(!A16 || (phases & 1) == 0 || (y == nullptr && y_rows != nullptr), "importance_qkv_x6_h16: fp16 rows are given as y_rows");
  PATHS_REQUIRE(B > 0 && N > 0 && N % 64 == 0 && D % 64 == 0 && D >= 256, "importance_qkv_x6: bad shape B=%d N=%d (a multiple of 64) D=%d", B, N, D);
  PATHS_REQUIRE(pe_mode == 1 || pe_mode == 2, "importance_qkv_x6: pe_mode must be 1 (1d) or 2 (2d)");
  PATHS_REQUIRE(pe_table != nullptr && pe_rows > 0 && (pe_mode == 1 || locs != nullptr), "importance_qkv_x6: needs the positional-encoding table (and locs in 2d mode)");
  PATHS_REQUIRE(num_ims != nullptr && splitk_ws != nullptr && (uintptr_t)splitk_ws % 16 == 0, "importance_qkv_x6: num_ims and a 16-byte aligned workspace are required");
  PATHS_REQUIRE(phases > 0 && (phases & ~7) == 0, "importance_qkv_x6: phases is a mask of 1 (GEMM), 2 (importance finish), 4 (tokens + in_proj finish)");
  PATHS_REQUIRE(pow2(w_scale) && pow2(a_scale), "importance_qkv_x6: scales must be powers of two");
  const int64_t M64 = (int64_t)B * N;
  PATHS_REQUIRE(M64 < (1ll << 24), "importance_qkv_x6: B * N must stay below 2^24 rows");
  const int M = (int)M64, T = N + 1, Tp = (T + 63) / 64 * 64;
  const int mt = (M + 127) / 128 * 4;
  const int64_t zstride = (int64_t)mt * 8 * 1024;
  if (phases & 1) {
    PATHS_REQUIRE(w_ip_x6 != nullptr && y_add != nullptr && (y != nullptr) != (y_rows != nullptr), "importance_qkv_x6: the GEMM takes (y or y_rows) + y_add");
    PATHS_REQUIRE(ldya % 4 == 0 && (uintptr_t)y_add % 16 == 0, "importance_qkv_x6: y_add must be 16-byte aligned with ldya %% 4 == 0");
    X6Operands g{y, ldy, D, y_rows, nullptr, 0, 0, y_add, ldya, reinterpret_cast<const char*>(w_ip_x6), group_stride(2, D), M, skip_padding ? num_ims : nullptr, N, a_scale};
    g.ksplit = 2;
    EpiRaw raw{splitk_ws, zstride, 8};
    int rc;
    if constexpr (A16) rc = launch_x6_np<2, 2, 4, 2, true, true, EpiRaw, 1, true>(g, 256, raw, stream, "importance_qkv_x6_h16(split-k)");
    else rc = y_rows ? launch_x6_np<2, 2, 4, 2, true, true>(g, 256, raw, stream, "importance_qkv_x6(split-k)")
                     : launch_x6_np<2, 2, 4, 2, true, false>(g, 256, raw, stream, "importance_qkv_x6(split-k)");
    if (rc != PATHS_OK) return rc;
  }
  if (phases & 6) {
    PATHS_REQUIRE(b1 && w2 && b2 && importance, "importance_qkv_x6: b1, w2, b2 (device scalar) and importance are required");
    FinQkvParams f{splitk_ws, zstride, 2, b1, w2, b2, bp, special, pe_table, pe_rows, locs, num_ims, N, T, Tp, B, patch_size, pe_mode, imp_mul,
                   skip_padding, 1.0f / (w_scale * a_scale), alpha_from_importance, importance, tokens, w_qkv, bqkv, 1.0f / s_wqkv, qscale, qkv_images,
                   (B % 8 == 0 && (M / 128) % 8 == 0 && M % 128 == 0) ? 1 : 0};
    if (phases & 2) {
      const int rc = paths_launch_finish_importance(f, stream);
      if (rc != PATHS_OK) return rc;
    }
    if (phases & 4) {
      PATHS_REQUIRE(bp && special && tokens && w_qkv && bqkv && qkv_images && pow2(s_wqkv), "importance_qkv_x6: null operand (tokens + in_proj finish)");
      PATHS_REQUIRE(((uintptr_t)tokens | (uintptr_t)w_qkv | (uintptr_t)qkv_images) % 16 == 0, "importance_qkv_x6: buffers must be 16-byte aligned");
      return paths_launch_finish_qkv(f, stream);
    }
  }
  return PATHS_OK;
}
}
extern "C" {

int paths_importance_qkv_x6(const float* y, int64_t ldy, const int64_t* y_rows, const float* y_add, int64_t ldya, const void* w_ip_x6,
                            const float* b1, const float* w2, const float* b2, const float* bp, const float* special,
                            const float* pe_table, int pe_rows, const int64_t* locs, const int64_t* num_ims, int B, int N,
                            int patch_size, int pe_mode, int imp_mul, float* importance, float* tokens, int D, int skip_padding,
                            float w_scale, float a_scale, float* splitk_ws, const void* w_qkv, const float* bqkv, float s_wqkv,
                            float qscale, void* qkv_images, int phases, int alpha_from_importance, hipStream_t stream) {
  return importance_qkv_x6<false>(y, ldy, y_rows, y_add, ldya, w_ip_x6, b1, w2, b2, bp, special, pe_table, pe_rows, locs, num_ims, B, N, patch_size,
                                  pe_mode, imp_mul, importance, tokens, D, skip_padding, w_scale, a_scale, splitk_ws, w_qkv, bqkv, s_wqkv, qscale,
                                  qkv_images, phases, alpha_from_importance, stream);
}

int paths_importance_qkv_x6_h16(const float* y, int64_t ldy, const int64_t* y_rows, const float* y_add, int64_t ldya, const void* w_ip_x6,
                                const float* b1, const float* w2, const float* b2, const float* bp, const float* special,
                                const float* pe_table, int pe_rows, const int64_t* locs, const int64_t* num_ims, int B, int N,
                                int patch_size, int pe_mode, int imp_mul, float* importance, float* tokens, int D, int skip_padding,
                                float w_scale, float a_scale, float* splitk_ws, const void* w_qkv, const float* bqkv, float s_wqkv,
                                float qscale, void* qkv_images, int phases, int alpha_from_importance, hipStream_t stream) {
  return importance_qkv_x6<true>(y, ldy, y_rows, y_add, ldya, w_ip_x6, b1, w2, b2, bp, special, pe_table, pe_rows, locs, num_ims, B, N, patch_size,
                                 pe_mode, imp_mul, importance, tokens, D, skip_padding, w_scale, a_scale, splitk_ws, w_qkv, bqkv, s_wqkv, qscale,
                                 qkv_images, phases, alpha_from_importance, stream);
}

#endif
#if PATHS_X6_PART == 0 || PATHS_X6_PART == 3
int paths_gemm_nt_x6(const float* a, int64_t lda, const void* w_x6, int Kpacked, int k0, const float* b, float* out, int64_t ldo,
                     int M, int N, int Npad, int K, int act, const float* residual, int64_t ldr, const float* mask,
                     int64_t ldm, int accumulate, int planes, float w_scale, float a_scale, hipStream_t stream) {
  PATHS_REQUIRE(k0 % 16 == 0 && k0 >= 0 && k0 + K <= Kpacked, "gemm_nt_x6: bad k window");
  PATHS_REQUIRE(planes == 3 || planes == 4 || (planes == 2 && pow2(w_scale) && pow2(a_scale)), "gemm_nt_x6: planes 3 / 4 (bf16), or planes 2 with power-of-two scales");
  if (planes != 2) w_scale = a_scale = 1.0f;
  X6Operands g{a, lda, K, nullptr, nullptr, 0, 0, nullptr, 0, reinterpret_cast<const char*>(w_x6) + (int64_t)(k0 / 16) * plane_count(planes) * FRAG, group_stride(planes, Kpacked), M, nullptr, 0, a_scale};
  EpiBias e{b, out, ldo, N, act, residual, ldr, mask, ldm, accumulate, 1.0f / (w_scale * a_scale)};
  if (Npad % 256 != 0) {
    if (planes == 4) return launch_x6_np<4, 2, 2, 2, false, false, EpiBias, 2>(g, Npad, e, stream, "gemm_nt_x6(n128, bf16 x 2)");
    if (planes == 3) return launch_x6_np<3, 2, 2, 2, false, false, EpiBias, 2>(g, Npad, e, stream, "gemm_nt_x6(n128)");
    return launch_x6_np<2, 2, 2, 2, false, false, EpiBias, 2>(g, Npad, e, stream, "gemm_nt_x6(n128)");
  }
  return launch_x6<2, 4, 2, false>(planes, g, Npad, e, stream, "gemm_nt_x6");
}

int paths_gemm_rows_nt_x6(const int64_t* a_rows, const void* w_x6, int Kpacked, int k0, float* out, int64_t ldo,
                          int M, int Npad, int K, int planes, float w_scale, float a_scale, hipStream_t stream) {
  PATHS_REQUIRE(a_rows != nullptr && planes == 2 && pow2(w_scale) && pow2(a_scale), "gemm_rows_nt_x6: row addresses need planes = 2 with power-of-two scales");
  PATHS_REQUIRE(k0 % 16 == 0 && k0 >= 0 && k0 + K <= Kpacked, "gemm_rows_nt_x6: bad k window");
  X6Operands g{nullptr, K, K, a_rows, nullptr, 0, 0, nullptr, 0,
               reinterpret_cast<const char*>(w_x6) + (int64_t)(k0 / 16) * planes * FRAG, group_stride(planes, Kpacked), M, nullptr, 0, a_scale};
  EpiBias e{nullptr, out, ldo, Npad, 0, nullptr, 0, nullptr, 0, 0, 1.0f / (w_scale * a_scale)};
  return launch_x6<2, 4, 2, false>(planes, g, Npad, e, stream, "gemm_rows_nt_x6");
}

int paths_gemm_add_nt_x6(const float* a, int64_t lda, const int64_t* a_rows, const float* a_add, int64_t ld_add, const void* w_x6, int Kpacked,
                         const float* b, float* out, int64_t ldo, int M, int N, int Npad, int K, int act, const int64_t* num_ims,
                         int rows_per_slide, float w_scale, float a_scale, hipStream_t stream) {
  PATHS_REQUIRE((a != nullptr) != (a_rows != nullptr), "gemm_add_nt_x6: exactly one of a / a_rows");
  PATHS_REQUIRE(a_add != nullptr && ld_add % 4 == 0 && (uintptr_t)a_add % 16 == 0, "gemm_add_nt_x6: a_add must be 16-byte aligned with ld_add %% 4 == 0");
  PATHS_REQUIRE(pow2(w_scale) && pow2(a_scale) && K == Kpacked && (Npad % 256 == 0 || Npad % 192 == 0),
                "gemm_add_nt_x6: power-of-two scales, whole-K image, Npad a multiple of 256 or of 192");
  X6Operands g{a, lda, K, a_rows, nullptr, 0, 0, a_add, ld_add, reinterpret_cast<const char*>(w_x6), group_stride(2, Kpacked), M, num_ims, rows_per_slide, a_scale};
  EpiBias e{b, out, ldo, N, act, nullptr, 0, nullptr, 0, 0, 1.0f / (w_scale * a_scale)};
  if (Npad % 256 != 0) {
    return a_rows ? launch_x6_np<2, 2, 3, 2, true, true>(g, Npad, e, stream, "gemm_add_nt_x6(rows, 192-wide tiles)")
                  : launch_x6_np<2, 2, 3, 2, true, false>(g, Npad, e, stream, "gemm_add_nt_x6(192-wide tiles)");
  }
  return a_rows ? launch_x6_np<2, 2, 4, 2, true, true>(g, Npad, e, stream, "gemm_add_nt_x6(rows)")
                : launch_x6_np<2, 2, 4, 2, true, false>(g, Npad, e, stream, "gemm_add_nt_x6");
}

int paths_gemm_add_nt_x6_h16(const float* a, int64_t lda, const int64_t* a_rows, const float* a_add, int64_t ld_add, const void* w_x6, int Kpacked,
                             const float* b, float* out, int64_t ldo, int M, int N, int Npad, int K, int act, const int64_t* num_ims,
                             int rows_per_slide, float w_scale, float a_scale, hipStream_t stream) {
  PATHS_REQUIRE(a == nullptr && a_rows != nullptr, "gemm_add_nt_x6_h16: fp16 rows are given as a_rows");
  PATHS_REQUIRE(a_add != nullptr && ld_add % 4 == 0 && (uintptr_t)a_add % 16 == 0, "gemm_add_nt_x6_h16: a_add must be 16-byte aligned with ld_add %% 4 == 0");
  PATHS_REQUIRE(pow2(w_scale) && pow2(a_scale) && K == Kpacked && (Npad % 256 == 0 || Npad % 192 == 0),
                "gemm_add_nt_x6_h16: power-of-two scales, whole-K image, Npad a multiple of 256 or of 192");
  X6Operands g{nullptr, lda, K, a_rows, nullptr, 0, 0, a_add, ld_add, reinterpret_cast<const char*>(w_x6), group_stride(2, Kpacked), M, num_ims, rows_per_slide, a_scale};
  EpiBias e{b, out, ldo, N, act, nullptr, 0, nullptr, 0, 0, 1.0f / (w_scale * a_scale)};
  if (Npad % 256 != 0) return launch_x6_np<2, 2, 3, 2, true, true, EpiBias, 1, true>(g, Npad, e, stream, "gemm_add_nt_x6_h16(rows, 192-wide tiles)");
  return launch_x6_np<2, 2, 4, 2, true, true, EpiBias, 1, true>(g, Npad, e, stream, "gemm_add_nt_x6_h16(rows)");
}

#endif

}
```

Measured before the change: 3898 slides/s.

## Pack ragged valid rows into GEMM tiles and drop forget gate at depth zero

New measurement: 3853 slides/s. 0.988x the previous value.

```diff
diff --git a/paths_amd/csrc/gemm_epi.h b/paths_amd/csrc/gemm_epi.h
--- a/paths_amd/csrc/gemm_epi.h
+++ b/paths_amd/csrc/gemm_epi.h
@@ -39,7 +39,24 @@
   else return trow + c32_row(r, lane) < M;
 }
 
+template <int WTM>
+struct TileRows {
+  int base[WTM]; unsigned live;
+  __device__ __forceinline__ bool on(int i) const { return (live >> i) & 1u; }
+};
+template <int WTM>
+__device__ __forceinline__ TileRows<WTM> linear_rows(int row0) {
+  TileRows<WTM> t;
+#pragma unroll
+  for (int i = 0; i < WTM; ++i) t.base[i] = row0 + 32 * i;
+  t.live = ~0u;
+  return t;
+}
+template <class E, class = void> struct epi_takes_rows : std::false_type {};
+template <class E> struct epi_takes_rows<E, std::void_t<decltype(E::takes_rows)>> : std::integral_constant<bool, E::takes_rows> {};
+
 struct EpiLstmC {
+  static constexpr bool takes_rows = true;
   const float* bias;
   const float* c0; int64_t ldc0;
   float* c1; int64_t ldc1;
@@ -48,20 +65,27 @@
   float acc_scale = 1.0f;
   template <int WTM, int WTN>
   __device__ __forceinline__ void init(f32x16 (&acc)[WTM][WTN], int row0, int col0, int lane, int M) const {
+    init_rows<WTM, WTN>(acc, linear_rows<WTM>(row0), col0, lane, M);
+  }
+  template <int WTM, int WTN>
+  __device__ __forceinline__ void init_rows(f32x16 (&acc)[WTM][WTN], const TileRows<WTM>& rows, int col0, int lane, int M) const {
     const int jj = lane & 31;
     const float seed = 1.0f / acc_scale;
-    if (hp == nullptr) {
+    if (hp == nullptr || WTN != 3) {
 #pragma unroll
       for (int i = 0; i < WTM; ++i)
 #pragma unroll
-        for (int r = 0; r < 16; ++r) { acc[i][0][r] = 0.f; acc[i][1][r] = 0.f; acc[i][2][r] = 0.f; }
+        for (int j = 0; j < WTN; ++j)
+#pragma unroll
+          for (int r = 0; r < 16; ++r) acc[i][j][r] = 0.f;
       return;
     }
+    if constexpr (WTN == 3) {
     int pr[WTM][16];
 #pragma unroll
     for (int i = 0; i < WTM; ++i)
 #pragma unroll
-      for (int r = 0; r < 16; ++r) pr[i][r] = hp_row[min(row0 + 32 * i + c32_row(r, lane), M - 1)];
+      for (int r = 0; r < 16; ++r) pr[i][r] = hp_row[min(rows.base[i] + c32_row(r, lane), M - 1)];
     float t[2][3][16];
     auto issue = [&](auto ic) __attribute__((always_inline)) {
       constexpr int i = decltype(ic)::value;
@@ -84,31 +108,36 @@
       }
     });
     __builtin_amdgcn_sched_barrier(0);
+    }
   }
   template <bool FULL, bool WITH_FRM, int WTM, int WTN>
-  __device__ __forceinline__ void run_impl(f32x16 (&acc)[WTM][WTN], int row0, int col0, int lane, int M) const {
+  __device__ __forceinline__ void run_impl(f32x16 (&acc)[WTM][WTN], const TileRows<WTM>& rows, int col0, int lane, int M) const {
     const int jj = lane & 31;
-    const int tcol = (col0 / 96) * 32;
-    const float bf = bias[col0 + jj], br = bias[col0 + 32 + jj], bm = bias[col0 + 64 + jj];
+    constexpr bool RM = WTN == 2;
+    const int ublk = RM ? col0 / 64 : col0 / 96;
+    const int tcol = ublk * 32, pcol = ublk * 96;
+    const float bf = RM ? 0.f : bias[pcol + jj], br = bias[pcol + 32 + jj], bm = bias[pcol + 64 + jj];
     const TileView c0v(c0, ldc0, lane), c1v(c1, ldc1, lane), fv(frm, ldfrm, lane);
     static_for<0, WTM>([&](auto ic) __attribute__((always_inline)) {
       constexpr int i = decltype(ic)::value;
-      const int trow = row0 + 32 * i;
-      char* o0 = c0v.tile(trow, tcol); char* o1 = c1v.tile(trow, tcol); char* of = fv.tile(trow, col0);
-      float cp[16];
-#pragma unroll
-      for (int r = 0; r < 16; ++r) cp[r] = c0 ? *tile_elem_o<FULL>(c0v, o0, trow, tcol, r, lane, M) : 0.f;
-#pragma unroll
-      for (int r = 0; r < 16; ++r) {
-        const float f = sigmoid_acc(fmaf(acc[i][0][r], acc_scale, bf));
-        const float rg = sigmoid_acc(fmaf(acc[i][1][r], acc_scale, br));
-        const float mp = tanh_acc(fmaf(acc[i][2][r], acc_scale, bm));
-        const float v = cp[r] * f + rg * mp;
-        if (tile_row_ok<FULL>(trow, r, lane, M)) {
-          *tile_elem_o<FULL>(c1v, o1, trow, tcol, r, lane, M) = v;
-          if constexpr (WITH_FRM) {
-            float* fr = tile_elem_o<FULL>(fv, of, trow, col0, r, lane, M);
-            fr[0] = f; fr[32] = rg; fr[64] = mp;
+      const int trow = rows.base[i];
+      if (rows.on(i)) {
+        char* o0 = c0v.tile(trow, tcol); char* o1 = c1v.tile(trow, tcol); char* of = fv.tile(trow, pcol);
+        float cp[16];
+#pragma unroll
+        for (int r = 0; r < 16; ++r) cp[r] = (c0 && !RM) ? *tile_elem_o<FULL>(c0v, o0, trow, tcol, r, lane, M) : 0.f;
+#pragma unroll
+        for (int r = 0; r < 16; ++r) {
+          const float f = RM ? 0.f : sigmoid_acc(fmaf(acc[i][0][r], acc_scale, bf));
+          const float rg = sigmoid_acc(fmaf(acc[i][RM ? 0 : 1][r], acc_scale, br));
+          const float mp = tanh_acc(fmaf(acc[i][RM ? 1 : 2][r], acc_scale, bm));
+          const float v = RM ? rg * mp : cp[r] * f + rg * mp;
+          if (tile_row_ok<FULL>(trow, r, lane, M)) {
+            *tile_elem_o<FULL>(c1v, o1, trow, tcol, r, lane, M) = v;
+            if constexpr (WITH_FRM && !RM) {
+              float* fr = tile_elem_o<FULL>(fv, of, trow, pcol, r, lane, M);
+              fr[0] = f; fr[32] = rg; fr[64] = mp;
+            }
           }
         }
       }
@@ -116,26 +145,34 @@
     });
   }
   template <int WTM, int WTN, int WGM, int WGN>
-  __device__ __forceinline__ void run(f32x16 (&acc)[WTM][WTN], int row0, int col0, int lane, int, int, int M, float*) const {
-    static_assert(WTN == 3, "LSTM c epilogue wants f|r|m tiles");
-    const bool full = row0 + 32 * WTM <= M;
+  __device__ __forceinline__ void run(f32x16 (&acc)[WTM][WTN], int row0, int col0, int lane, int wm, int wn, int M, float* smem) const {
+    run_rows<WTM, WTN, WGM, WGN>(acc, linear_rows<WTM>(row0), row0 + 32 * WTM <= M, col0, lane, wm, wn, M, smem);
+  }
+  template <int WTM, int WTN, int WGM, int WGN>
+  __device__ __forceinline__ void run_rows(f32x16 (&acc)[WTM][WTN], const TileRows<WTM>& rows, bool full, int col0, int lane, int, int, int M, float*) const {
+    static_assert(WTN == 3 || WTN == 2, "LSTM c epilogue wants f|r|m tiles (r|m at depth 0)");
     if (frm == nullptr) {
-      if (full) run_impl<true, false>(acc, row0, col0, lane, M);
-      else run_impl<false, false>(acc, row0, col0, lane, M);
+      if (full) run_impl<true, false>(acc, rows, col0, lane, M);
+      else run_impl<false, false>(acc, rows, col0, lane, M);
     } else {
-      if (full) run_impl<true, true>(acc, row0, col0, lane, M);
-      else run_impl<false, true>(acc, row0, col0, lane, M);
+      if (full) run_impl<true, true>(acc, rows, col0, lane, M);
+      else run_impl<false, true>(acc, rows, col0, lane, M);
     }
   }
 };
 
 template <bool RAW>
 struct EpiLstmO_ {
+  static constexpr bool takes_rows = RAW;
   const float* bias; float* o; int64_t ldo; int N;
   const float* hp; int64_t ldhp; const int* hp_row; int hp_col0;
   float acc_scale = 1.0f;
   template <int WTM, int WTN>
   __device__ __forceinline__ void init(f32x16 (&acc)[WTM][WTN], int row0, int col0, int lane, int M) const {
+    init_rows<WTM, WTN>(acc, linear_rows<WTM>(row0), col0, lane, M);
+  }
+  template <int WTM, int WTN>
+  __device__ __forceinline__ void init_rows(f32x16 (&acc)[WTM][WTN], const TileRows<WTM>& rows, int col0, int lane, int M) const {
     const float seed = 1.0f / acc_scale;
     if (hp == nullptr) {
 #pragma unroll
@@ -150,7 +187,7 @@
 #pragma unroll
     for (int i = 0; i < WTM; ++i)
 #pragma unroll
-      for (int r = 0; r < 16; ++r) pr[i][r] = hp_row[min(row0 + 32 * i + c32_row(r, lane), M - 1)];
+      for (int r = 0; r < 16; ++r) pr[i][r] = hp_row[min(rows.base[i] + c32_row(r, lane), M - 1)];
     float t[2][WTN][16];
     auto issue = [&](auto ic) __attribute__((always_inline)) {
       constexpr int i = decltype(ic)::value;
@@ -175,12 +212,12 @@
     __builtin_amdgcn_sched_barrier(0);
   }
   template <bool FULL, int WTM, int WTN>
-  __device__ __forceinline__ void run_impl(f32x16 (&acc)[WTM][WTN], int row0, int col0, int lane, int M) const {
+  __device__ __forceinline__ void run_impl(f32x16 (&acc)[WTM][WTN], const TileRows<WTM>& rows, int col0, int lane, int M) const {
     const TileView ov(o, ldo, lane);
     static_for<0, WTM * WTN>([&](auto tc) __attribute__((always_inline)) {
       constexpr int t = decltype(tc)::value, i = t % WTM, j = t / WTM;
-      const int trow = row0 + 32 * i, tcol = col0 + 32 * j;
-      if (tcol < N) {
+      const int trow = rows.base[i], tcol = col0 + 32 * j;
+      if (tcol < N && rows.on(i)) {
         const float b = bias[tcol + (lane & 31)];
         char* origin = ov.tile(trow, tcol);
 #pragma unroll
@@ -192,7 +229,11 @@
     });
   }
   template <int WTM, int WTN, int WGM, int WGN>
-  __device__ __forceinline__ void run(f32x16 (&acc)[WTM][WTN], int row0, int col0, int lane, int, int, int M, float*) const {
+  __device__ __forceinline__ void run(f32x16 (&acc)[WTM][WTN], int row0, int col0, int lane, int wm, int wn, int M, float* smem) const {
+    run_rows<WTM, WTN, WGM, WGN>(acc, linear_rows<WTM>(row0), row0 + 32 * WTM <= M, col0, lane, wm, wn, M, smem);
+  }
+  template <int WTM, int WTN, int WGM, int WGN>
+  __device__ __forceinline__ void run_rows(f32x16 (&acc)[WTM][WTN], const TileRows<WTM>& rows, bool full, int col0, int lane, int, int, int M, float*) const {
     if constexpr (RAW) {
       const int ntn = N >> 5;
 #pragma unroll
@@ -202,7 +243,8 @@
           const float b = bias[tcol + (lane & 31)];
 #pragma unroll
           for (int i = 0; i < WTM; ++i) {
-            f32x4* t = reinterpret_cast<f32x4*>(o + ((int64_t)((row0 >> 5) + i) * ntn + (tcol >> 5)) * 1024) + lane;
+            if (!rows.on(i)) continue;
+            f32x4* t = reinterpret_cast<f32x4*>(o + ((int64_t)(rows.base[i] >> 5) * ntn + (tcol >> 5)) * 1024) + lane;
 #pragma unroll
             for (int q = 0; q < 4; ++q)
               t[64 * q] = f32x4{fmaf(acc[i][j][4 * q], acc_scale, b), fmaf(acc[i][j][4 * q + 1], acc_scale, b),
@@ -211,8 +253,8 @@
         }
       }
     } else {
-      if (row0 + 32 * WTM <= M) run_impl<true>(acc, row0, col0, lane, M);
-      else run_impl<false>(acc, row0, col0, lane, M);
+      if (full) run_impl<true>(acc, rows, col0, lane, M);
+      else run_impl<false>(acc, rows, col0, lane, M);
     }
   }
 };
@@ -221,6 +263,9 @@
 
 template <bool WITH_Y, bool WITH_TC = false, bool RAW_O = false>
 struct EpiLstmH {
+  static constexpr bool takes_rows = RAW_O && !WITH_Y && !WITH_TC;
+  template <int WTM, int WTN>
+  __device__ __forceinline__ void init_rows(f32x16 (&acc)[WTM][WTN], const TileRows<WTM>&, int col0, int lane, int M) const { init<WTM, WTN>(acc, 0, col0, lane, M); }
   template <int WTM, int WTN>
   __device__ __forceinline__ void init(f32x16 (&acc)[WTM][WTN], int, int, int, int) const {
 #pragma unroll
@@ -236,13 +281,13 @@
   float* tc_out;
   float acc_scale = 1.0f;
   template <bool FULL, int WTM, int WTN>
-  __device__ __forceinline__ void run_impl(f32x16 (&acc)[WTM][WTN], int row0, int col0, int lane, int M) const {
+  __device__ __forceinline__ void run_impl(f32x16 (&acc)[WTM][WTN], const TileRows<WTM>& rows, int col0, int lane, int M) const {
     constexpr int NT = WTM * WTN, PD = (NT >= 4 && !WITH_Y) ? 3 : 1, NB = PD + 1;
     const TileView ovw(o, ldo, lane), xvw(x, ldx, lane), hv(h1, ldh, lane), yv(y, ldy, lane), tv(tc_out, N, lane);
     float ov[NB][16], xv[WITH_Y ? NB : 1][16];
     auto load = [&](auto tc) __attribute__((always_inline)) {
       constexpr int t = decltype(tc)::value, i = t % WTM, j = t / WTM, s = t % NB;
-      const int trow = row0 + 32 * i, tcol = min(col0 + 32 * j, N - 32);
+      const int trow = rows.base[i], tcol = min(col0 + 32 * j, N - 32);
       char* to = ovw.tile(trow, tcol); char* tx = xvw.tile(trow, tcol);
       if constexpr (RAW_O) {
         const f32x4* t4 = reinterpret_cast<const f32x4*>(o + ((int64_t)(trow >> 5) * (N >> 5) + (tcol >> 5)) * 1024) + lane;
@@ -267,8 +312,8 @@
     static_for<0, NT>([&](auto tc) __attribute__((always_inline)) {
       constexpr int t = decltype(tc)::value, i = t % WTM, j = t / WTM, s = t % NB;
       if constexpr (t + PD < NT) load(std::integral_constant<int, t + PD>{});
-      const int trow = row0 + 32 * i, tcol = col0 + 32 * j;
-      if (tcol < N) {
+      const int trow = rows.base[i], tcol = col0 + 32 * j;
+      if (tcol < N && rows.on(i)) {
         const float b = bias[tcol + (lane & 31)];
         char* th = hv.tile(trow, tcol); char* ty = yv.tile(trow, tcol); char* tt = tv.tile(trow, tcol);
         static_for<0, 16>([&](auto rc) __attribute__((always_inline)) {
@@ -290,9 +335,13 @@
     });
   }
   template <int WTM, int WTN, int WGM, int WGN>
-  __device__ __forceinline__ void run(f32x16 (&acc)[WTM][WTN], int row0, int col0, int lane, int, int, int M, float*) const {
-    if (row0 + 32 * WTM <= M) run_impl<true>(acc, row0, col0, lane, M);
-    else run_impl<false>(acc, row0, col0, lane, M);
+  __device__ __forceinline__ void run(f32x16 (&acc)[WTM][WTN], int row0, int col0, int lane, int wm, int wn, int M, float* smem) const {
+    run_rows<WTM, WTN, WGM, WGN>(acc, linear_rows<WTM>(row0), row0 + 32 * WTM <= M, col0, lane, wm, wn, M, smem);
+  }
+  template <int WTM, int WTN, int WGM, int WGN>
+  __device__ __forceinline__ void run_rows(f32x16 (&acc)[WTM][WTN], const TileRows<WTM>& rows, bool full, int col0, int lane, int, int, int M, float*) const {
+    if (full) run_impl<true>(acc, rows, col0, lane, M);
+    else run_impl<false>(acc, rows, col0, lane, M);
   }
 };
 
@@ -478,6 +527,7 @@
       const int nslides = M / rows_per_slide;
       const int nim0 = (int)num_ims[b0], nim1 = (int)num_ims[min(b0 + 1, nslides - 1)];
       int tokrow[16]; float av[16]; bool first[16]; float pev[16][2];
+      unsigned vld = 0u;
 #pragma unroll
       for (int r = 0; r < 16; ++r) {
         const int lrow = wm * WTM * 32 + 32 * i + c32_row(r, lane);
@@ -492,7 +542,7 @@
           b = small_rows ? div_u24(row, rows_per_slide, rps_inv) : row / rows_per_slide; idx = row - b * rows_per_slide; nim = (int)num_ims[b];
         }
         float a = 0.f;
-        if (idx < nim) a = sigmoid_acc((alpha_p[lrow] + alpha_p[RB + lrow]) + b2v);
+        if (idx < nim) { a = sigmoid_acc((alpha_p[lrow] + alpha_p[RB + lrow]) + b2v); vld |= 1u << r; }
         if (wn == 0 && (lane & 31) == 0 && rowr < M) importance[rowr] = a;
         av[r] = imp_mul ? a : 1.f;
         tokrow[r] = b * (rows_per_slide + 1) + idx + 1;
@@ -525,7 +575,7 @@
           for (int j = 0; j < 2; ++j) {
             const int c = u0 + 32 * j + (lane & 31);
             const float pj = acc[i][2 + j][r] * acc_scale;
-            trow[c] = av[r] * pj + bpv[j] + pev[r][j];
+            trow[c] = av[r] * (((vld >> r) & 1u) ? pj : 0.f) + bpv[j] + pev[r][j];
             if constexpr (SAVE) pproj_out[(int64_t)row * 128 + c] = pj;
             if (first[r]) trow[c - d] = spv[j];
           }
diff --git a/paths_amd/csrc/gemm_x6.hip b/paths_amd/csrc/gemm_x6.hip
--- a/paths_amd/csrc/gemm_x6.hip
+++ b/paths_amd/csrc/gemm_x6.hip
@@ -2,6 +2,7 @@
 #include "gemm_epi.h"
 #include "finish_qkv.h"
 #include "split.h"
+#include "ragged_rows.h"
 
 #ifndef PATHS_X6_PART
 #define PATHS_X6_PART 0
@@ -26,7 +27,10 @@
   int rows_per_slide;
   float a_scale;
   int ksplit = 1;
+  int w_rm = 0;
+  int pack_rows = 0;
 };
+constexpr int ROW_GRANULE = 64;
 
 template <int NP, int WTM, int WTN, int PF, bool ADD, bool ROWS, class Epi, int OCC = 1, bool A16 = false>
 __global__ void __launch_bounds__(256) __attribute__((amdgpu_waves_per_eu(OCC, OCC)))
@@ -56,7 +60,24 @@
   const int rows_in_grp = min(GM, nby - grp * GM);
   const int by = grp * GM + in_grp % rows_in_grp, bx = in_grp / rows_in_grp;
   const int m0 = by * BM, n0 = bx * BN;
-  if (block_all_padding(g.num_ims, g.rows_per_slide, m0, BM, g.M)) return;
+  constexpr bool CAN_PACK = epi_takes_rows<Epi>::value && NP == 2;
+  const bool packed = CAN_PACK && g.pack_rows != 0;
+  int grow0[BM / ROW_GRANULE]; unsigned glive = ~0u;
+  if (packed) {
+    int gr[BM / ROW_GRANULE];
+    ragged_rows_granules(g.num_ims, g.M / g.rows_per_slide, g.rows_per_slide, ROW_GRANULE, by * (BM / ROW_GRANULE), gr);
+    if (gr[0] < 0) return;
+    glive = 0u;
+#pragma unroll
+    for (int p = 0; p < BM / ROW_GRANULE; ++p) {
+      if (gr[p] >= 0) glive |= 1u << p;
+      grow0[p] = gr[p] >= 0 ? gr[p] : gr[0];
+    }
+  } else {
+    if (block_all_padding(g.num_ims, g.rows_per_slide, m0, BM, g.M)) return;
+#pragma unroll
+    for (int p = 0; p < BM / ROW_GRANULE; ++p) grow0[p] = m0 + p * ROW_GRANULE;
+  }
 
   const int arow = tid >> 2, ac = tid & 3;
   uint32_t aoff0[NA], aoff1[NA], aoffs[ADD ? NA : 1]; int awr[NA];
@@ -67,7 +88,7 @@
 #pragma unroll
   for (int p = 0; p < NA; ++p) {
     const int row = p * 64 + arow;
-    const int64_t grow = min(m0 + row, g.M - 1);
+    const int64_t grow = min(grow0[p] + arow, g.M - 1);
     aoff0[p] = ROWS ? 0u : (uint32_t)((grow * g.lda0 + 4 * ac) * 4);
     if constexpr (A16) rowh[p] = reinterpret_cast<gptr_h4>(static_cast<uintptr_t>(g.A0rows[grow]) + 8 * ac);
     else if constexpr (ROWS) rowp[p] = reinterpret_cast<gptr_f4>(static_cast<uintptr_t>(g.A0rows[grow]) + 16 * ac);
@@ -93,7 +114,8 @@
     int pc = wave + 4 * i;
     if (pc >= NPB) pc -= 4;
     const int sub = pc / PL, pl = pc % PL;
-    bbase[i] = g.Wt + ((int64_t)(n0 >> 5) + sub) * g.w_group_stride + pl * FRAG;
+    const int st = (n0 >> 5) + sub;
+    bbase[i] = g.Wt + (int64_t)(g.w_rm ? 3 * (st >> 1) + 1 + (st & 1) : st) * g.w_group_stride + pl * FRAG;
     bwr[i] = (A1P ? SA * SUBTA + sub * SUBT : (SA + sub) * SUBT) + pl * FRAG + lane * 16;
   }
   static_assert(PF == 1 || PF == 2, "one or two register sets");
@@ -198,7 +220,14 @@
   auto swrite_b = [&](int set, int q, int buf) { *reinterpret_cast<u32x4*>(smem + buf * STAGE + bwr[q]) = sbr[set][q]; };
 
   f32x16 acc[WTM][WTN];
-  epi.template init<WTM, WTN>(acc, m0 + wm * WTM * 32, n0 + wn * WTN * 32, lane, g.M);
+  TileRows<WTM> trows;
+#pragma unroll
+  for (int i = 0; i < WTM; ++i) trows.base[i] = (wm ? grow0[WTM / 2 + i / 2] : grow0[i / 2]) + 32 * (i & 1);
+  trows.live = 0u;
+#pragma unroll
+  for (int i = 0; i < WTM; ++i) trows.live |= ((glive >> (wm * (WTM / 2) + i / 2)) & 1u) << i;
+  if constexpr (CAN_PACK) epi.template init_rows<WTM, WTN>(acc, trows, n0 + wn * WTN * 32, lane, g.M);
+  else epi.template init<WTM, WTN>(acc, m0 + wm * WTM * 32, n0 + wn * WTN * 32, lane, g.M);
 
   const char* sA = smem + (wm * WTM) * SUBTA + lane * 16;
   const char* sB = A1P ? smem + SA * SUBTA + (wn * WTN) * SUBT + lane * 16 : smem + (SA + wn * WTN) * SUBT + lane * 16;
@@ -335,7 +364,12 @@
   stage_body(nk - 2, I0, T, F);
   stage_body(nk - 1, I1, F, F);
   __syncthreads();
-  epi.template run<WTM, WTN, 2, 2>(acc, m0 + wm * WTM * 32, n0 + wn * WTN * 32, lane, wm, wn, g.M, reinterpret_cast<float*>(smem));
+  if constexpr (CAN_PACK) {
+    const bool full = packed || m0 + (wm + 1) * WTM * 32 <= g.M;
+    epi.template run_rows<WTM, WTN, 2, 2>(acc, trows, full, n0 + wn * WTN * 32, lane, wm, wn, g.M, reinterpret_cast<float*>(smem));
+  } else {
+    epi.template run<WTM, WTN, 2, 2>(acc, m0 + wm * WTM * 32, n0 + wn * WTN * 32, lane, wm, wn, g.M, reinterpret_cast<float*>(smem));
+  }
 }
 
 template <int NP>
@@ -399,6 +433,8 @@
   auto kern = gemm_x6_kernel<NP, WTM, WTN, PF, ADD, ROWS, Epi, OCC, A16>;
   PATHS_LDS_OPT_IN(kern, lds, name);
   PATHS_REQUIRE(g.ksplit == 1 || (g.ksplit > 1 && g.K1 == 0 && g.K0 % (32 * g.ksplit) == 0 && g.K0 / g.ksplit >= 128), "%s: split-K needs a single panel and k windows that are multiples of 32, >= 128", name);
+  PATHS_REQUIRE(!g.pack_rows || (epi_takes_rows<Epi>::value && NP == 2 && g.num_ims != nullptr && g.rows_per_slide > 0 && g.rows_per_slide % ROW_GRANULE == 0 && g.M % g.rows_per_slide == 0),
+                "%s: packed rows need the two-plane split, an epilogue that takes row bases, num_ims and whole slides of a multiple of %d rows", name, ROW_GRANULE);
   dim3 grid(Npad / BN, (g.M + BM - 1) / BM, g.ksplit);
   hipLaunchKernelGGL(kern, grid, dim3(256), lds, stream, g, epi);
   PATHS_LAUNCH_CHECK(name);
@@ -406,8 +442,11 @@
 }
 
 struct EpiRaw {
+  static constexpr bool takes_rows = true;
   float* ws; int64_t zstride; int ntn;
   template <int WTM, int WTN>
+  __device__ __forceinline__ void init_rows(f32x16 (&acc)[WTM][WTN], const TileRows<WTM>&, int col0, int lane, int M) const { init<WTM, WTN>(acc, 0, col0, lane, M); }
+  template <int WTM, int WTN>
   __device__ __forceinline__ void init(f32x16 (&acc)[WTM][WTN], int, int, int, int) const {
 #pragma unroll
     for (int i = 0; i < WTM; ++i)
@@ -417,13 +456,18 @@
         for (int r = 0; r < 16; ++r) acc[i][j][r] = 0.f;
   }
   template <int WTM, int WTN, int WGM, int WGN>
-  __device__ __forceinline__ void run(f32x16 (&acc)[WTM][WTN], int row0, int col0, int lane, int, int, int, float*) const {
+  __device__ __forceinline__ void run(f32x16 (&acc)[WTM][WTN], int row0, int col0, int lane, int wm, int wn, int M, float* smem) const {
+    run_rows<WTM, WTN, WGM, WGN>(acc, linear_rows<WTM>(row0), true, col0, lane, wm, wn, M, smem);
+  }
+  template <int WTM, int WTN, int WGM, int WGN>
+  __device__ __forceinline__ void run_rows(f32x16 (&acc)[WTM][WTN], const TileRows<WTM>& rows, bool, int col0, int lane, int, int, int, float*) const {
     float* base = ws + (int64_t)blockIdx.z * zstride;
 #pragma unroll
     for (int i = 0; i < WTM; ++i)
 #pragma unroll
       for (int j = 0; j < WTN; ++j) {
-        f32x4* t = reinterpret_cast<f32x4*>(base + ((int64_t)((row0 >> 5) + i) * ntn + (col0 >> 5) + j) * 1024) + lane;
+        if (!rows.on(i)) continue;
+        f32x4* t = reinterpret_cast<f32x4*>(base + ((int64_t)(rows.base[i] >> 5) * ntn + (col0 >> 5) + j) * 1024) + lane;
 #pragma unroll
         for (int q = 0; q < 4; ++q) {
           const f32x4 v = f32x4{acc[i][j][4 * q], acc[i][j][4 * q + 1], acc[i][j][4 * q + 2], acc[i][j][4 * q + 3]};
@@ -534,10 +578,22 @@
   const float sg = 1.0f / (wg_scale * a_scale), sm = 1.0f / (wm_scale * a_scale);
   X6Operands g{x, ldx, D, x_rows, h0, h0 ? ldh0 : 0, h0 ? D : 0, nullptr, 0, wg, gs, M, num_ims, rows_per_slide, a_scale};
   const bool small_m = planes == 2 && M <= 8192 && (h0 == nullptr);
+  const bool o_raw = y == nullptr && save_tc == nullptr && save_frm == nullptr;
+  const int pack = (o_raw && planes == 2 && num_ims != nullptr && rows_per_slide > 0 && rows_per_slide % ROW_GRANULE == 0 && M % rows_per_slide == 0) ? 1 : 0;
+  g.pack_rows = pack;
   if (phases & 1) {
     EpiLstmC e{b_gates, c0, ldc0, state_out + D, ldso, save_frm, (int64_t)3 * Hc, hp, (int64_t)3 * Hc + D, hp_row, sg};
     int rc;
-    if constexpr (A16) {
+    if (o_raw && planes == 2 && c0 == nullptr && hp == nullptr && h0 == nullptr) {
+      X6Operands grm = g; grm.w_rm = 1;
+      if constexpr (A16) {
+        rc = small_m ? launch_x6_np<2, 2, 2, 2, false, true, decltype(e), 1, true>(grm, 2 * Hc, e, stream, "lstm_cell_x6_h16(c, r|m, 128-row tiles)")
+                     : launch_x6_np<2, 4, 2, 1, false, true, decltype(e), 1, true>(grm, 2 * Hc, e, stream, "lstm_cell_x6_h16(c, r|m)");
+      } else if (small_m) rc = x_rows ? launch_x6_np<2, 2, 2, 2, false, true>(grm, 2 * Hc, e, stream, "lstm_cell_x6(c, r|m, 128-row tiles)")
+                               : launch_x6_np<2, 2, 2, 2, false, false>(grm, 2 * Hc, e, stream, "lstm_cell_x6(c, r|m, 128-row tiles)");
+      else rc = x_rows ? launch_x6_np<2, 4, 2, 1, false, true>(grm, 2 * Hc, e, stream, "lstm_cell_x6(c, r|m)")
+                       : launch_x6_np<2, 4, 2, 1, false, false>(grm, 2 * Hc, e, stream, "lstm_cell_x6(c, r|m)");
+    } else if constexpr (A16) {
       rc = small_m ? launch_x6_np<2, 2, 3, 2, false, true, decltype(e), 1, true>(g, 3 * Hc, e, stream, "lstm_cell_x6_h16(c, 128-row tiles)")
                    : launch_x6_np<2, 4, 3, 1, false, true, decltype(e), 1, true>(g, 3 * Hc, e, stream, "lstm_cell_x6_h16(c)");
     } else if (small_m) rc = x_rows ? launch_x6_np<2, 2, 3, 2, false, true>(g, 3 * Hc, e, stream, "lstm_cell_x6(c, 128-row tiles)")
@@ -545,7 +601,6 @@
     else rc = launch_x6<4, 3, 1, false>(planes, g, 3 * Hc, e, stream, "lstm_cell_x6(c)");
     if (rc) return rc;
   }
-  const bool o_raw = y == nullptr && save_tc == nullptr && save_frm == nullptr;
   if (phases & 2) {
     X6Operands go = g;
     go.Wt = wg + (int64_t)(3 * Hc / 32) * gs;
@@ -567,6 +622,7 @@
   }
   if (phases & 4) {
     X6Operands gh{state_out + D, ldso, Hc, nullptr, nullptr, 0, 0, nullptr, 0, reinterpret_cast<const char*>(w_mem_x6), group_stride(planes, Hc), M, num_ims, rows_per_slide, a_scale};
+    gh.pack_rows = pack;
     int rc;
     PATHS_REQUIRE(save_tc == nullptr || y != nullptr, "lstm_cell_x6: save_tc (training) needs y");
     PATHS_REQUIRE(planes == 2 || planes == 3, "lstm_cell_x6: planes must be 3 (bf16 x6) or 2 (fp16 x3), got %d", planes);
@@ -646,13 +702,14 @@
       if (splitk_ws != nullptr && planes == 2 && (y_add != nullptr || y_rows == nullptr) && D % 64 == 0 && D >= 256) {
         const int mt = (M + 127) / 128 * 4;
         const int64_t zstride = (int64_t)mt * 8 * 1024;
+        const int pack = (skip_padding && save_hid == nullptr && rows_per_slide % ROW_GRANULE == 0) ? 1 : 0;
         int rc;
         if constexpr (A16) {
-          X6Operands gs = g; gs.ksplit = 2;
+          X6Operands gs = g; gs.ksplit = 2; gs.pack_rows = pack;
           EpiRaw raw{splitk_ws, zstride, 8};
           rc = launch_x6_np<2, 2, 4, 2, true, true, EpiRaw, 1, true>(gs, 256, raw, stream, "importance_proj_x6_h16(split-k)");
         } else {
-          X6Operands gs = g; gs.ksplit = 2;
+          X6Operands gs = g; gs.ksplit = 2; gs.pack_rows = pack;
           EpiRaw raw{splitk_ws, zstride, 8};
           rc = y_add == nullptr ? launch_x6_np<2, 2, 4, 2, false, false>(gs, 256, raw, stream, "importance_proj_x6(split-k, stored y)")
                : y_rows ? launch_x6_np<2, 2, 4, 2, true, true>(gs, 256, raw, stream, "importance_proj_x6(split-k)")
@@ -728,6 +785,7 @@
     PATHS_REQUIRE(ldya % 4 == 0 && (uintptr_t)y_add % 16 == 0, "importance_qkv_x6: y_add must be 16-byte aligned with ldya %% 4 == 0");
     X6Operands g{y, ldy, D, y_rows, nullptr, 0, 0, y_add, ldya, reinterpret_cast<const char*>(w_ip_x6), group_stride(2, D), M, skip_padding ? num_ims : nullptr, N, a_scale};
     g.ksplit = 2;
+    g.pack_rows = skip_padding ? 1 : 0;
     EpiRaw raw{splitk_ws, zstride, 8};
     int rc;
     if constexpr (A16) rc = launch_x6_np<2, 2, 4, 2, true, true, EpiRaw, 1, true>(g, 256, raw, stream, "importance_qkv_x6_h16(split-k)");
diff --git a/paths_amd/csrc/ragged_rows.h b/paths_amd/csrc/ragged_rows.h
--- /dev/null
+++ b/paths_amd/csrc/ragged_rows.h
@@ -0,0 +1,38 @@
+#pragma once
+#include <stdint.h>
+
+#if defined(__HIPCC__) || defined(__CUDACC__)
+#define PATHS_RAGGED_HD __host__ __device__
+#else
+#define PATHS_RAGGED_HD
+#endif
+
+template <int NG>
+PATHS_RAGGED_HD inline int ragged_rows_granules(const int64_t* num_ims, int B, int N, int G, int g0, int (&rows)[NG]) {
+  if (num_ims == nullptr || N % G != 0) {
+    const int64_t M = (int64_t)B * N;
+    const int total = (int)((M + G - 1) / G);
+    for (int k = 0; k < NG; ++k) rows[k] = (g0 + k >= 0 && g0 + k < total) ? (g0 + k) * G : -1;
+    return total;
+  }
+  for (int k = 0; k < NG; ++k) rows[k] = -1;
+  int before = 0;
+  for (int b = 0; b < B; ++b) {
+    const int64_t n64 = num_ims[b];
+    const int n = n64 < 0 ? 0 : n64 > N ? N : (int)n64;
+    const int cnt = (n + G - 1) / G;
+    for (int k = 0; k < NG; ++k) {
+      const int q = g0 + k - before;
+      if (q >= 0 && q < cnt) rows[k] = b * N + q * G;
+    }
+    before += cnt;
+  }
+  return before;
+}
+
+PATHS_RAGGED_HD inline int ragged_rows_granule(const int64_t* num_ims, int B, int N, int G, int g, int* total) {
+  int row[1];
+  const int t = ragged_rows_granules<1>(num_ims, B, N, G, g, row);
+  if (total != nullptr) *total = t;
+  return row[0];
+}
```
